# dpkn31/Yade-OpenFOAM-coupling

Measured on AMD Instinct MI355X. Metric: coupled_steps_per_sec (pimpleFoamYade 4-way, 10M particles / 4M cells per GPU), higher is better.
Workload: dtype f64

## Files before the change

yade-openfoam-coupling_amd/csrc/common.hpp:

```cpp
#pragma once
#include <hip/hip_runtime.h>

#include <algorithm>
#include <cmath>
#include <cstdarg>
#include <cstdint>
#include <cstdio>
#include <cstring>
#include <string>
#include <vector>

#include "../../include/foamyade_hip.h"

namespace fy {

struct Options {
    std::string tree_cache_dir;
    int rebin_interval;
    int strip_blocks;
    bool halo_overlap;
    int ipc_slot_mb;
    long long ipc_timeout_ms;
    bool wire_trace;
    bool explicit_tree;
    bool no_locate_lists;
    int locate_stack;
    bool locate_wide;
    bool no_deep_vcycle;
    long long mg_replicate_below;
    int amg_passes;
    bool localcomm_stream;
    bool no_fused_corrector;
    bool faces_from_arrays;
    bool no_pairs;
    bool no_tail_cache;
    int ipc_slot_kb;
};
Options options();

std::string& last_error();
int fail(int code, const char* fmt, ...);
bool pairs_disabled();
bool tail_cache_disabled();
bool locate_wide_forced();

#define FY_HIP(expr)                                                                                      \
    do {                                                                                                  \
        hipError_t _e = (expr);                                                                           \
        if (_e != hipSuccess)                                                                             \
            return ::fy::fail(FY_ERR_HIP, "%s failed: %s (%s:%d)", #expr, hipGetErrorString(_e), __FILE__, __LINE__); \
    } while (0)

#define FY_TRY(expr)                 \
    do {                             \
        int _rc = (expr);            \
        if (_rc != FY_OK) return _rc; \
    } while (0)

template <class T>
struct DevBuf {
    T* p = nullptr;
    size_t n = 0;
    DevBuf() = default;
    DevBuf(const DevBuf&) = delete;
    DevBuf& operator=(const DevBuf&) = delete;
    ~DevBuf() { release(); }
    void release() {
        if (p) (void)hipFree(p);
        p = nullptr;
        n = 0;
    }
    int reserve(size_t count) {
        if (count <= n) return FY_OK;
        release();
        size_t cap = count + count / 8 + 64;
        hipError_t e = hipMalloc((void**)&p, cap * sizeof(T));
        if (e != hipSuccess) {
            p = nullptr;
            return fail(FY_ERR_HIP, "hipMalloc(%zu bytes) failed: %s", cap * sizeof(T), hipGetErrorString(e));
        }
        n = cap;
        return FY_OK;
    }
    int alloc_exact(size_t count) {
        release();
        if (count == 0) return FY_OK;
        hipError_t e = hipMalloc((void**)&p, count * sizeof(T));
        if (e != hipSuccess) {
            p = nullptr;
            return fail(FY_ERR_HIP, "hipMalloc(%zu bytes) failed: %s", count * sizeof(T), hipGetErrorString(e));
        }
        n = count;
        return FY_OK;
    }
};

template <class T>
struct HostBuf {
    T* p = nullptr;
    size_t n = 0;
    HostBuf() = default;
    HostBuf(const HostBuf&) = delete;
    HostBuf& operator=(const HostBuf&) = delete;
    ~HostBuf() { release(); }
    void release() {
        if (p) (void)hipHostFree(p);
        p = nullptr;
        n = 0;
    }
    T* data() { return p; }
    T& operator[](size_t i) { return p[i]; }
    int reserve(size_t count) {
        if (count <= n) return FY_OK;
        release();
        const size_t cap = count + count / 8 + 64;
        hipError_t e = hipHostMalloc((void**)&p, cap * sizeof(T), hipHostMallocDefault);
        if (e != hipSuccess) {
            p = nullptr;
// ... 141 lines not shown
```

yade-openfoam-coupling_amd/csrc/coupling.cpp:

```cpp
#include "coupling.hpp"
#include "ldu.hpp"

#include <algorithm>
#include <cmath>
#include <chrono>
#include <cstdlib>
#include <functional>
#include <thread>

#include <sys/stat.h>
#include <unistd.h>

#include <atomic>

namespace fy {

static std::atomic<int> g_kernel_flags{-1};
static bool kernel_flag(int bit) {
    if (g_kernel_flags.load(std::memory_order_relaxed) < 0) (void)options();
    return (g_kernel_flags.load(std::memory_order_relaxed) >> bit) & 1;
}
bool pairs_disabled() { return kernel_flag(0); }
bool tail_cache_disabled() { return kernel_flag(1); }
bool locate_wide_forced() { return kernel_flag(2); }

Options options() {
    auto on = [](const char* nm) { const char* e = getenv(nm); return e != nullptr && *e != 0 && strcmp(e, "0") != 0; };
    auto num = [](const char* nm, long long unset) { const char* e = getenv(nm); return e ? atoll(e) : unset; };
    Options q{};
    if (const char* d = getenv("FOAMYADE_TREE_CACHE_DIR")) q.tree_cache_dir = d;
    q.rebin_interval = std::max(1, (int)num("FOAMYADE_REBIN_INTERVAL", 32));
    q.strip_blocks = (int)num("FOAMYADE_STRIP_BLOCKS", -1);
    q.halo_overlap = getenv("FOAMYADE_HALO_OVERLAP") == nullptr || on("FOAMYADE_HALO_OVERLAP");
    q.ipc_slot_mb = (int)num("FOAMYADE_IPC_SLOT_MB", 0);
    q.ipc_timeout_ms = num("FOAMYADE_IPC_TIMEOUT_MS", 0);
    q.wire_trace = getenv("FOAMYADE_WIRE_TRACE") != nullptr;
    q.explicit_tree = on("FOAMYADE_EXPLICIT_TREE");
    q.no_locate_lists = on("FOAMYADE_NO_LOCATE_LISTS");
    q.locate_stack = (int)num("FOAMYADE_LOCATE_STACK", -1);
    q.locate_wide = num("FOAMYADE_LOCATE_WIDE", 0) != 0;
    q.no_deep_vcycle = on("FOAMYADE_NO_DEEP_VCYCLE");
    q.mg_replicate_below = std::max(0LL, num("FOAMYADE_MG_REPLICATE_BELOW", 0));
    q.amg_passes = (int)std::min(3LL, std::max(1LL, num("FOAMYADE_AMG_PASSES", 3)));
    const char* ls = getenv("FOAMYADE_LOCALCOMM_STREAM");
    q.localcomm_stream = ls != nullptr && ls[0] == '1';
    q.no_fused_corrector = on("FOAMYADE_NO_FUSED_CORRECTOR");
    q.faces_from_arrays = on("FOAMYADE_FACES_FROM_ARRAYS");
    q.no_pairs = on("FOAMYADE_NO_PAIRS");
    q.no_tail_cache = on("FOAMYADE_NO_TAIL_CACHE");
    q.ipc_slot_kb = (int)num("FOAMYADE_IPC_SLOT_KB", 0);
    g_kernel_flags.store((q.no_pairs ? 1 : 0) | (q.no_tail_cache ? 2 : 0) | (q.locate_wide ? 4 : 0), std::memory_order_relaxed);
    return q;
}

std::string& last_error() {
    static thread_local std::string e;
    return e;
}

int fail(int code, const char* fmt, ...) {
    char buf[1024];
    va_list ap;
    va_start(ap, fmt);
    vsnprintf(buf, sizeof(buf), fmt, ap);
    va_end(ap);
    last_error() = buf;
    return code;
}

static const int TAG_SZ_BUFF = 1003, TAG_GRID_BBOX = 1001, TAG_YADE_DATA = 1002, TAG_FORCE = 1005, TAG_SEARCH_RES = 1004,
                 TAG_FLUID_DT = 1050, TAG_YADE_DT = 1060;

#define FY_TR(expr)                                                                             \
    do {                                                                                        \
        if ((expr) != 0) return fail(FY_ERR_TRANSPORT, "transport call failed: %s", #expr);     \
    } while (0)

int Coupling::create(const fy_mesh_desc* m, const fy_field_ptrs* f, int gaussian_interp, const fy_transport* tr, int device_ordinal) {
    if (!m || !f || m->n_cells <= 0 || !m->centres || !m->volumes) return fail(FY_ERR_INVALID, "fy_create: bad mesh/fields");
    int ndev = 0;
    if (hipGetDeviceCount(&ndev) != hipSuccess || ndev == 0)
        return fail(FY_ERR_NO_DEVICE, "no HIP device visible: libfoamyade_hip has no CPU path");
    if (device_ordinal < 0 || device_ordinal >= ndev) return fail(FY_ERR_INVALID, "device ordinal %d out of range (%d devices)", device_ordinal, ndev);
    device = device_ordinal;
    opt = options();
    FY_HIP(hipSetDevice(device));
    if (ext_stream) { stream = ext_stream; owns_stream = false; }
    else { FY_HIP(hipStreamCreate(&stream)); owns_stream = true; }
    mesh = *m;
    mesh.centres = nullptr; mesh.volumes = nullptr; mesh.xf = mesh.yf = mesh.zf = nullptr;
    n_cells = m->n_cells;
    gaussian = gaussian_interp != 0;
    structured = m->nx > 0;
    rectilinear = structured && m->xf && m->yf && m->zf;
    if (!gaussian && !structured && !ldu_geo) return fail(FY_ERR_UNSUPPORTED, "point-force mode needs the structured block description, or a general mesh's face addressing (fy_ldu_solver): the findCell stand-ins");
    if (structured && (int64_t)m->nx * m->ny * m->nz != m->n_cells) return fail(FY_ERR_INVALID, "nx*ny*nz != n_cells");
    if (tr) { transport = *tr; has_transport = true; }

    if (has_transport) {
        comm_sz_diff = std::abs(transport.world_size - transport.local_size);
        serial_yade = (comm_sz_diff == 1);
    } else {
        comm_sz_diff = 0; serial_yade = true;
    }

    {
        bool exact = structured && !rectilinear && !opt.explicit_tree && m->nx <= 1024 && m->ny <= 1024 && m->nz <= 4096 &&
                     n_cells < (1 << 25);
        if (exact)
            for (int k = 0; k < m->nz && exact; ++k) for (int j = 0; j < m->ny && exact; ++j) for (int i = 0; i < m->nx; ++i) {
                const size_t c = (size_t)i + (size_t)m->nx * (j + (size_t)m->ny * k);
                const double x = m->origin[0] + ((double)i + 0.5) * m->dx, y = m->origin[1] + ((double)j + 0.5) * m->dx, z = m->origin[2] + ((double)k + 0.5) * m->dx;
                if (x != m->centres[3 * c] || y != m->centres[3 * c + 1] || z != m->centres[3 * c + 2]) { exact = false; break; }
            }
        std::vector<int32_t> pre;
        std::string cache;
        const std::string& cache_dir = opt.tree_cache_dir;
        if (exact && !cache_dir.empty()) {
            char nm[512];
            snprintf(nm, sizeof(nm), "%s/fy_tree_%dx%dx%d_%016llx.bin", cache_dir.c_str(), m->nx, m->ny, m->nz,
                     (unsigned long long)(std::hash<double>()(m->dx) ^ (std::hash<double>()(m->origin[0]) << 1) ^ (std::hash<double>()(m->origin[1]) << 2) ^ (std::hash<double>()(m->origin[2]) << 3)));
            cache = nm;
        }
        auto load_cache = [&]() -> bool {
            FILE* f = fopen(cache.c_str(), "rb");
            if (!f) return false;
            pre.resize((size_t)n_cells);
            bool ok = fread(pre.data(), sizeof(int32_t), (size_t)n_cells, f) == (size_t)n_cells && fgetc(f) == EOF;
            fclose(f);
            for (size_t q = 0; ok && q < pre.size(); ++q) ok = pre[q] >= 0 && pre[q] < n_cells;
            if (!ok) pre.clear();
            return ok;
// ... 1306 lines not shown
```

yade-openfoam-coupling_amd/csrc/fv_kernels.hip:

```cpp
#include "fv_kernels.hpp"

#include "common.hpp"
#include "device_util.hpp"
#include "fv_closures.hpp"

#ifndef FY_FVK_GRADED
#define FY_FVK_GRADED 0
#endif

namespace fy {
#if FY_FVK_GRADED
namespace gr {
#endif
namespace {

constexpr double kSmall = 1e-15;

__device__ __forceinline__ void ijk_of(const FvGeo& g, int t, int& i, int& j, int& k) {
    i = t % g.nx;
    const int q = t / g.nx;
    j = q % g.ny;
    k = q / g.ny;
}
__device__ __forceinline__ int cidx(const FvGeo& g, int i, int j, int k) { return i + g.nx * (j + g.ny * (k + g.gz)); }
// ... 1270 lines not shown
#pragma unroll
        for (int d = 0; d < 3; ++d)
#pragma unroll
            for (int s = 0; s < 2; ++s) {
                pn[d][s] = p[nb[d][s]];
                phh[d][s] = phiHbyA.a[d][fx[d][s]];
                pfo[d][s] = pim ? phiForces.a[d][fx[d][s]] : 0.0;
                if (FFC) { rfv[d][s] = rAU[nb[d][s]]; afv[d][s] = pim ? alpha[nb[d][s]] : 1.0; }
                else { rfv[d][s] = rAUf.arr.a[d][fx[d][s]]; afv[d][s] = pim ? alphaf.arr.a[d][fx[d][s]] : 1.0; }
            }
        double pfl[3][2], ph[3][2];
#pragma unroll
        for (int d = 0; d < 3; ++d)
#pragma unroll
            for (int s = 0; s < 2; ++s) {
                const int q = ijk[d] + s;
                const int fi = i + (d == 0 ? s : 0), fj = j + (d == 1 ? s : 0), fk = k + (d == 2 ? s : 0);
                const bool b = bnd[d][s];
                if (FFC) {
                    afv[d][s] = pim ? (b ? 1.0 : lerp_face(g, d, s, q, ac, afv[d][s])) : 1.0;
                    rfv[d][s] = b ? rc : lerp_face(g, d, s, q, rc, rfv[d][s]);
                }
                const double af = afv[d][s], rf = rfv[d][s];
                double fl = 0.0;
                if (b) {
                    const int patch = 2 * d + s;
                    if (g.p_bc[patch] == 1) { const double gb = kBfac * af * rf * geo_sfd_face(g, d, q, ndim(g, d), fi, fj, fk); fl = s ? gb * (g.p_val[patch] - pc) : gb * (pc - g.p_val[patch]); }
                    else if (g.p_bc[patch] == 2) fl = af * rf * geo_Af(g, d, fi, fj, fk) * psn.a[d][fx[d][s]];
                } else {
                    fl = af * rf * geo_sfd_face(g, d, q, ndim(g, d), fi, fj, fk) * (s ? pn[d][s] - pc : pc - pn[d][s]);
                }
                const double fa = fl / af;
                pfl[d][s] = pim ? (pfo[d][s] - fa) / rf : fl;
                ph[d][s] = phh[d][s] - fa;
                if (owns_face(g, d, s, i, j, k)) phi.a[d][fx[d][s]] = ph[d][s];
            }
        double out[3];
        double dv = 0.0, sp = 0.0;
#pragma unroll
        for (int d = 0; d < 3; ++d) {
            if (!pim) {
                double fv[2];
#pragma unroll
                for (int s = 0; s < 2; ++s) {
                    if (bnd[d][s]) fv[s] = pbv(g, p, psn, c, d, s, fx[d][s]);
                    else fv[s] = geo_lerp_side(g, d, s, ijk[d], pc, pn[d][s]);
                }
                out[d] = hb[d] - rc * ((fv[1] - fv[0]) * geo_rh(g, d, ijk[d]));
            } else {
                double sm = 0;
#pragma unroll
                for (int s = 0; s < 2; ++s) sm += pfl[d][s];
                out[d] = hb[d] + rc * (sm / (2.0 * geo_Af(g, d, i, j, k)));
            }
            if (DIAG) {
#pragma unroll
                for (int s = 0; s < 2; ++s) {
                    dv += (s ? 1.0 : -1.0) * (pim ? afv[d][s] : 1.0) * ph[d][s];
                    sp += fabs(ph[d][s]);
                }
            }
        }
        for (int d = 0; d < 3; ++d) U[3 * (size_t)c + d] = out[d];
        if (DIAG) {
            double ce = dv * geo_rV(g, i, j, k);
            if (pim) ce += (ac - alphaOld[c]) / g.dt;
            v[0] += fabs(ce) * geo_V(g, i, j, k);
            v[1] += ce * geo_V(g, i, j, k);
            v[2] = fmax(v[2], sp * geo_rV(g, i, j, k));
            v[3] += sp;
        }
    }
    if (DIAG) {
        const int mx[4] = {0, 0, 1, 0};
        block_reduce_store<4>(v, mx, partials, fy_lb, fy_stride);
    }
}

template <bool STORE_A, bool FFC>
__global__ __launch_bounds__(256) __attribute__((amdgpu_waves_per_eu(4))) void k_corr_front(FvGeo g, const double* __restrict__ HbyA, const double* __restrict__ U, CFace3 dcorr,
                                                    FaceSrc rAUf, FaceSrc alphaf, CFace3 phiForces, Face3 phiHbyA, Face3 psn,
                                                    const double* __restrict__ rAU, const double* __restrict__ alpha, const double* __restrict__ alphaOld, PMat A,
                                                    double* __restrict__ rhs, const double* __restrict__ x, const double* __restrict__ xbar_dev, double xsum_val,
                                                    double inv_n, double* __restrict__ res, double* __restrict__ partials) {
    double v[2] = {0, 0};
    const double xbar = (xbar_dev ? xbar_dev[0] : xsum_val) * inv_n;
    FY_RED_LOOP_G(g, t) {
        int i, j, k; ijk_of(g, t, i, j, k);
        const int c = t + g.c0;
        const int ijk[3] = {i, j, k};
        const bool pim = g.pimple != 0;
        const bool refc = g.need_ref && (i + g.nx * (j + g.ny * (k + g.kglob0))) == g.p_ref_cell;
        bool bnd[3][2]; int nb[3][2], fx[3][2];
#pragma unroll
        for (int d = 0; d < 3; ++d)
#pragma unroll
            for (int s = 0; s < 2; ++s) {
                bnd[d][s] = onb(g, d, s, i, j, k);
                nb[d][s] = bnd[d][s] ? c : c + (s ? stride_of(g, d) : -stride_of(g, d));
                fx[d][s] = cface(g, d, s, i, j, k);
            }
        const double xc = x[c], ac = pim ? alpha[c] : 1.0;
        const double rc = FFC ? rAU[c] : 0.0;
        const double hb[3] = {HbyA[3 * (size_t)c], HbyA[3 * (size_t)c + 1], HbyA[3 * (size_t)c + 2]};
        double hn[3][2], dc[3][2], pfo[3][2], xn[3][2], rfv[3][2], afv[3][2];
#pragma unroll
        for (int d = 0; d < 3; ++d)
#pragma unroll
            for (int s = 0; s < 2; ++s) {
                hn[d][s] = HbyA[3 * (size_t)nb[d][s] + d];
                dc[d][s] = dcorr.a[d][fx[d][s]];
                pfo[d][s] = pim ? phiForces.a[d][fx[d][s]] : 0.0;
                xn[d][s] = x[nb[d][s]];
                if (FFC) { rfv[d][s] = rAU[nb[d][s]]; afv[d][s] = pim ? alpha[nb[d][s]] : 1.0; }
                else { rfv[d][s] = rAUf.arr.a[d][fx[d][s]]; afv[d][s] = pim ? alphaf.arr.a[d][fx[d][s]] : 1.0; }
            }
        double dg = 0.0, r = 0.0, up[3] = {0, 0, 0};
        double gg6[3][2];
#pragma unroll
        for (int d = 0; d < 3; ++d)
#pragma unroll
            for (int s = 0; s < 2; ++s) {
                const int q = ijk[d] + s;
                const int fi = i + (d == 0 ? s : 0), fj = j + (d == 1 ? s : 0), fk = k + (d == 2 ? s : 0);
                const bool b = bnd[d][s];
                const int patch = 2 * d + s;
                if (FFC) {
                    afv[d][s] = pim ? (b ? 1.0 : lerp_face(g, d, s, q, ac, afv[d][s])) : 1.0;
                    rfv[d][s] = b ? rc : lerp_face(g, d, s, q, rc, rfv[d][s]);
                }
                const double af = afv[d][s], rf = rfv[d][s];
                const double Afc = geo_Af(g, d, fi, fj, fk);
                double pv = (b ? ub_normal(g, patch, d, hb[d]) : lerp_face(g, d, s, q, hb[d], hn[d][s])) * Afc;
                double add = rf * dc[d][s];
                if (pim) add *= af;
                pv += add;
                if (pim) pv += pfo[d][s];
                const bool own = owns_face(g, d, s, i, j, k);
                if (own) phiHbyA.a[d][fx[d][s]] = pv;
                double ph = (s ? 1.0 : -1.0) * af * pv;
                gg6[d][s] = 0.0;
                if (b) {
                    if (g.p_bc[patch] == 2) {
                        const double ubd = ub_normal(g, patch, d, g.u_bc[patch] == 1 ? U[3 * (size_t)c + d] : 0.0);
                        const double psn_v = (pv - ubd * Afc) / (rf * Afc);
                        if (own) psn.a[d][fx[d][s]] = psn_v;
                        ph = (s ? 1.0 : -1.0) * af * (pv - rf * geo_Af(g, d, i, j, k) * psn_v);
                    }
                    r -= ph;
                    if (g.p_bc[patch] == 1) { const double gb = kBfac * af * rf * geo_sfd(g, d, s, i, j, k); dg += gb; r += gb * g.p_val[patch]; }
                } else {
                    r -= ph;
                    const double gg = af * rf * geo_sfd(g, d, s, i, j, k);
                    dg += gg; gg6[d][s] = gg;
                    if (s) up[d] = gg;
                }
            }
        if (pim) r -= geo_V(g, i, j, k) * (ac - alphaOld[c]) / g.dt;
        if (refc) { r += dg * g.p_ref_value; dg += dg; }
        if (STORE_A) { A.diag[c] = dg; A.ux[c] = up[0]; A.uy[c] = up[1]; A.uz[c] = up[2]; }
        rhs[c] = r;
        double Ax = dg * xc, rs = dg;
#pragma unroll
        for (int d = 0; d < 3; ++d)
#pragma unroll
            for (int s = 0; s < 2; ++s)
                if (!bnd[d][s]) { Ax -= gg6[d][s] * xn[d][s]; rs -= gg6[d][s]; }
        const double Aref = rs * xbar;
        const double rr = r - Ax;
        res[c] = rr;
        v[0] += fabs(rr);
        v[1] += fabs(Ax - Aref) + fabs(r - Aref);
    }
    const int mx[2] = {0, 0};
    block_reduce_store<2>(v, mx, partials, fy_lb, fy_stride);
}

__device__ __forceinline__ bool bface_side(const FvGeo& g, int b, int& side, int& r) {
    const int nyz = g.ny * g.nz, nxz = g.nx * g.nz, nxy = g.nx * g.ny;
    if (b < 2 * nyz) { side = b >= nyz; r = b - side * nyz; return true; }
    b -= 2 * nyz;
    if (b < 2 * nxz) { const int s = b >= nxz; side = 2 + s; r = b - s * nxz; return true; }
    b -= 2 * nxz;
    if (b < 2 * nxy) { const int s = b >= nxy; side = 4 + s; r = b - s * nxy; return true; }
    return false;
}
__device__ __forceinline__ double Tbv(const TPatch& e, const double* T, int c, int patch) { return e.bc[patch] == 1 ? e.val[patch] : T[c]; }
struct BFace { double A, phi, p, ux, uy, uz, T; };
template <int D, int S>
__device__ __forceinline__ void bface_values(const FvGeo& g, int r, int want, const double* __restrict__ p, const double* psn_d, const double* __restrict__ U,
                                             const double* __restrict__ T, const TPatch& te, const double* phi_d, BFace& o) {
    CFace3 psn{};
    psn.a[D] = psn_d;
    int i, j, k;
    if (D == 0) { j = r % g.ny; k = r / g.ny; i = S ? g.nx - 1 : 0; }
    else if (D == 1) { i = r % g.nx; k = r / g.nx; j = S ? g.ny - 1 : 0; }
    else { i = r % g.nx; j = r / g.nx; k = S ? g.nz - 1 : 0; }
    const int c = cidx(g, i, j, k), face = cface(g, D, S, i, j, k), patch = 2 * D + S;
    o.A = geo_Af(g, D, i, j, k);
    if (want & (1 << MF_PHI)) o.phi = (S ? 1.0 : -1.0) * phi_d[face];
    if (want & (1 << MF_P)) o.p = pbv(g, p, psn, c, D, S, face);
    if (want & (7 << MF_U)) { double u[3]; Ub(g, U, c, patch, u); o.ux = u[0]; o.uy = u[1]; o.uz = u[2]; }
    if (want & (1 << MF_T)) o.T = Tbv(te, T, c, patch);
}
__device__ __forceinline__ void bface_values_of(const FvGeo& g, int side, int r, int want, const double* __restrict__ p, CFace3 psn, const double* __restrict__ U,
                                                const double* __restrict__ T, const TPatch& te, CFace3 phi, BFace& o) {
    switch (side) {
        case 0: bface_values<0, 0>(g, r, want, p, psn.a[0], U, T, te, phi.a[0], o); break;
        case 1: bface_values<0, 1>(g, r, want, p, psn.a[0], U, T, te, phi.a[0], o); break;
        case 2: bface_values<1, 0>(g, r, want, p, psn.a[1], U, T, te, phi.a[1], o); break;
        case 3: bface_values<1, 1>(g, r, want, p, psn.a[1], U, T, te, phi.a[1], o); break;
        case 4: bface_values<2, 0>(g, r, want, p, psn.a[2], U, T, te, phi.a[2], o); break;
        default: bface_values<2, 1>(g, r, want, p, psn.a[2], U, T, te, phi.a[2], o); break;
    }
}

__global__ __launch_bounds__(256) void k_boundary_values(FvGeo g, const double* __restrict__ p, CFace3 psn, const double* __restrict__ U, const double* __restrict__ T, TPatch te,
                                                         double* __restrict__ pb, double* __restrict__ ub, double* __restrict__ tb) {
    const int b = blockIdx.x * 256 + threadIdx.x;
    int side, r;
    if (!bface_side(g, b, side, r)) return;
    BFace v{};
    bface_values_of(g, side, r, (pb ? 1 << MF_P : 0) | (ub ? 7 << MF_U : 0) | (tb ? 1 << MF_T : 0), p, psn, U, T, te, CFace3{}, v);
    if (pb) pb[b] = v.p;
    if (ub) { ub[3 * (size_t)b] = v.ux; ub[3 * (size_t)b + 1] = v.uy; ub[3 * (size_t)b + 2] = v.uz; }
    if (tb) tb[b] = v.T;
}

__global__ __launch_bounds__(256) void k_monitor_faces(FvGeo g, MonFaceTable t, const double* __restrict__ p, CFace3 psn, const double* __restrict__ U, const double* __restrict__ T,
                                                       TPatch te, CFace3 phi, double* __restrict__ partials) {
    const MonFaceObj o = t.o[blockIdx.y];
    const int b = blockIdx.x * 256 + threadIdx.x;
    int side = 0, r = 0;
    bool in = bface_side(g, b, side, r);
    in = in && ((o.patch >> side) & 1);
    BFace v{};
    if (in) bface_values_of(g, side, r, o.fields | (1 << MF_PHI), p, psn, U, T, te, phi, v);
    const double x[kMonFaceComps] = {1.0, v.phi, v.p, v.ux, v.uy, v.uz, v.T};
    const int slot0 = (int)blockIdx.y * kMonFaceComps * kMonKinds;
#pragma unroll
    for (int q = 0; q < kMonFaceComps; ++q) {
        if (!((o.fields >> q) & 1)) continue;
        double w[kMonKinds];
        mon_terms(in, x[q], v.A, v.phi, w);
        mon_block_reduce_store(w, partials, slot0 + q * kMonKinds, (int)gridDim.x, (int)blockIdx.x);
    }
}

inline int fv_grid(const FvGeo& g) { return g.win_nblk > 0 ? g.win_nblk : div_up(g.Nc, 256); }
inline int fv_red_grid(const FvGeo& g) { return g.win_nblk > 0 ? g.win_nblk : red_blocks(g.Nc); }

}

// ... 111 lines not shown

int launch_HbyA(hipStream_t s, FvGeo g, Mom7 M, const double* src, const double* U, const double* rAU, double* HbyA) {
    hipLaunchKernelGGL(k_HbyA, dim3(fv_grid(g)), dim3(256), 0, s, g, M, src, U, rAU, HbyA);
    FY_LAUNCH_CHECK();
    return FY_OK;
}

int launch_phiHbyA(hipStream_t s, FvGeo g, const double* HbyA, const double* U, const double* Uold, CFace3 phiOld, CFace3 rAUf,
                   CFace3 alphaf, CFace3 phiForces, Face3 out, Face3 psn, Face3 ddtc, int keep) {
    if (keep == 1) hipLaunchKernelGGL(k_phiHbyA_cells<1>, dim3(fv_grid(g)), dim3(256), 0, s, g, HbyA, U, Uold, phiOld, rAUf, alphaf, phiForces, out, psn, ddtc);
    else if (keep == 2) hipLaunchKernelGGL(k_phiHbyA_cells<2>, dim3(fv_grid(g)), dim3(256), 0, s, g, HbyA, U, Uold, phiOld, rAUf, alphaf, phiForces, out, psn, ddtc);
    else hipLaunchKernelGGL(k_phiHbyA_cells<0>, dim3(fv_grid(g)), dim3(256), 0, s, g, HbyA, U, Uold, phiOld, rAUf, alphaf, phiForces, out, psn, ddtc);
    FY_LAUNCH_CHECK();
    return FY_OK;
}

int launch_adjust_phi_sums(hipStream_t s, FvGeo g, CFace3 phiHbyA, CFace3 phiForces, double* partials) {
    hipLaunchKernelGGL(k_adjust_phi_sums, dim3(fv_red_grid(g)), dim3(256), 0, s, g, phiHbyA, phiForces, partials);
    FY_LAUNCH_CHECK();
    return FY_OK;
}

int launch_adjust_phi_apply(hipStream_t s, FvGeo g, const double* sums, Face3 phiHbyA, CFace3 phiForces, CFace3 rAUf, const double* U, Face3 psn, int* err) {
    const size_t nbf = 2 * ((size_t)g.ny * g.nz + (size_t)g.nx * g.nz + (size_t)g.nx * g.ny);
    hipLaunchKernelGGL(k_adjust_phi_apply, dim3(div_up(nbf, 256)), dim3(256), 0, s, g, sums, phiHbyA, phiForces, rAUf, U, psn, err);
    FY_LAUNCH_CHECK();
    return FY_OK;
}

int launch_rAUf_phi_forces(hipStream_t s, FvGeo g, const double* rAU, const double* uSource, Face3 rf, Face3 out) {
    hipLaunchKernelGGL(k_rAUf_phi_forces_cells, dim3(fv_grid(g)), dim3(256), 0, s, g, rAU, uSource, rf, out);
    FY_LAUNCH_CHECK();
    return FY_OK;
}

int launch_assemble_pressure(hipStream_t s, FvGeo g, CFace3 phiHbyA, CFace3 rAUf, CFace3 alphaf, CFace3 psn, const double* alpha,
                             const double* alphaOld, PMat A, double* rhs, bool matrix) {
    if (matrix) hipLaunchKernelGGL(k_assemble_pressure<true>, dim3(fv_grid(g)), dim3(256), 0, s, g, phiHbyA, rAUf, alphaf, psn, alpha, alphaOld, A, rhs);
    else hipLaunchKernelGGL(k_assemble_pressure<false>, dim3(fv_grid(g)), dim3(256), 0, s, g, phiHbyA, rAUf, alphaf, psn, alpha, alphaOld, A, rhs);
    FY_LAUNCH_CHECK();
    return FY_OK;
}

int launch_flux_correct(hipStream_t s, FvGeo g, const double* p, CFace3 phiHbyA, CFace3 rAUf, CFace3 alphaf, CFace3 psn, CFace3 phiForces, Face3 pflux, Face3 phi) {
    hipLaunchKernelGGL(k_flux_correct_cells, dim3(fv_grid(g)), dim3(256), 0, s, g, p, phiHbyA, rAUf, alphaf, psn, phiForces, pflux, phi);
    FY_LAUNCH_CHECK();
    return FY_OK;
}

int launch_cont_err(hipStream_t s, FvGeo g, CFace3 phi, CFace3 alphaf, const double* alpha, const double* alphaOld, double* partials) {
    hipLaunchKernelGGL(k_cont_err, dim3(fv_red_grid(g)), dim3(256), 0, s, g, phi, alphaf, alpha, alphaOld, partials);
    FY_LAUNCH_CHECK();
    return FY_OK;
}

int launch_U_correct(hipStream_t s, FvGeo g, const double* HbyA, const double* rAU, const double* p, CFace3 psn, CFace3 phiForces,
                     CFace3 pflux, CFace3 alphaf, CFace3 rAUf, double* U) {
    hipLaunchKernelGGL(k_U_correct<false>, dim3(fv_red_grid(g)), dim3(256), 0, s, g, HbyA, rAU, p, psn, phiForces, pflux, alphaf, rAUf, U, CFace3{}, nullptr, nullptr, nullptr);
    FY_LAUNCH_CHECK();
    return FY_OK;
}

int launch_U_correct_diag(hipStream_t s, FvGeo g, const double* HbyA, const double* rAU, const double* p, CFace3 psn, CFace3 phiForces,
                          CFace3 pflux, CFace3 alphaf, CFace3 rAUf, double* U, CFace3 phi, const double* alpha, const double* alphaOld, double* partials) {
    hipLaunchKernelGGL(k_U_correct<true>, dim3(fv_red_grid(g)), dim3(256), 0, s, g, HbyA, rAU, p, psn, phiForces, pflux, alphaf, rAUf, U, phi, alpha, alphaOld, partials);
    FY_LAUNCH_CHECK();
    return FY_OK;
}

int launch_corr_back(hipStream_t s, FvGeo g, const double* p, CFace3 phiHbyA, CFace3 rAUf, CFace3 alphaf, CFace3 psn, CFace3 phiForces, Face3 phi,
                     const double* HbyA, const double* rAU, double* U, const double* alpha, const double* alphaOld, double* partials, bool faces_from_cells) {
    const FaceSrc rs{rAUf, faces_from_cells ? rAU : nullptr}, as{alphaf, faces_from_cells ? alpha : nullptr};
    const dim3 grid(fv_red_grid(g)), blk(256);
#define FY_BACK(DG, FC) hipLaunchKernelGGL((k_corr_back<DG, FC>), grid, blk, 0, s, g, p, phiHbyA, rs, as, psn, phiForces, phi, HbyA, rAU, U, alpha, alphaOld, partials)
    if (partials) { if (faces_from_cells) FY_BACK(true, true); else FY_BACK(true, false); }
    else { if (faces_from_cells) FY_BACK(false, true); else FY_BACK(false, false); }
#undef FY_BACK
    FY_LAUNCH_CHECK();
    return FY_OK;
}

int launch_corr_front(hipStream_t s, FvGeo g, const double* HbyA, const double* U, CFace3 dcorr, CFace3 rAUf, CFace3 alphaf, CFace3 phiForces, Face3 phiHbyA,
                      Face3 psn, const double* rAU, const double* alpha, const double* alphaOld, PMat A, double* rhs, bool store_A, const double* x,
                      const double* xsum_dev, double xsum_val, double inv_n, double* res, double* partials, bool faces_from_cells) {
    const FaceSrc rs{rAUf, faces_from_cells ? rAU : nullptr}, as{alphaf, faces_from_cells ? alpha : nullptr};
    const dim3 grid(fv_red_grid(g)), blk(256);
#define FY_FRONT(SA, FC) hipLaunchKernelGGL((k_corr_front<SA, FC>), grid, blk, 0, s, g, HbyA, U, dcorr, rs, as, phiForces, phiHbyA, psn, rAU, alpha, alphaOld, A, rhs, \
                                            x, xsum_dev, xsum_val, inv_n, res, partials)
    if (store_A) { if (faces_from_cells) FY_FRONT(true, true); else FY_FRONT(true, false); }
    else { if (faces_from_cells) FY_FRONT(false, true); else FY_FRONT(false, false); }
#undef FY_FRONT
    FY_LAUNCH_CHECK();
    return FY_OK;
}

int launch_p_ghost_uz(hipStream_t s, FvGeo g, CFace3 rAUf, CFace3 alphaf, PMat A) {
    hipLaunchKernelGGL(k_p_ghost_uz, dim3(div_up((size_t)g.nx * g.ny, 256)), dim3(256), 0, s, g, rAUf, alphaf, A);
    FY_LAUNCH_CHECK();
    return FY_OK;
}

int launch_boundary_values(hipStream_t s, FvGeo g, const double* p, CFace3 psn, const double* U, const double* T, TPatch te, double* pb, double* ub, double* tb) {
    const size_t nb = 2 * ((size_t)g.ny * g.nz + (size_t)g.nx * g.nz + (size_t)g.nx * g.ny);
    hipLaunchKernelGGL(k_boundary_values, dim3(div_up(nb, 256)), dim3(256), 0, s, g, p, psn, U, T, te, pb, ub, tb);
    FY_LAUNCH_CHECK();
    return FY_OK;
}

int launch_monitor_faces(hipStream_t s, FvGeo g, MonFaceTable t, const double* p, CFace3 psn, const double* U, const double* T, TPatch te, CFace3 phi, double* partials, int nblk) {
    if (t.n <= 0) return FY_OK;
    hipLaunchKernelGGL(k_monitor_faces, dim3(nblk, t.n), dim3(256), 0, s, g, t, p, psn, U, T, te, phi, partials);
    FY_LAUNCH_CHECK();
    return FY_OK;
}

#if FY_FVK_GRADED
}
#endif
}
```

yade-openfoam-coupling_amd/csrc/fv_kernels_api.inc:

```

int launch_flux_of(hipStream_t s, FvGeo g, const double* F, Face3 out);
int launch_courant(hipStream_t s, FvGeo g, CFace3 phi, double* partials);
int launch_pre_coupling(hipStream_t s, FvGeo g, const double* U, const double* p, const double* alpha, CFace3 psn,
                        double* vGrad, double* gradP, double* divT, double* Gout, int write_vgrad, int write_pfields,
                        CFace3 phi = CFace3{}, double* ddtU = nullptr, double* Uold_out = nullptr,
                        double* cellrec = nullptr ,
                        double rec_nu = 0.0, double rec_rhoF = 0.0,
                        Face3 dcorr = Face3{} );
int launch_interp_alpha(hipStream_t s, FvGeo g, const double* alpha, Face3 alphaf);
int launch_div_G(hipStream_t s, FvGeo g, const double* G, double* divG);
int launch_assemble_turb(hipStream_t s, FvGeo g, TurbEqn e, const double* k, const double* eps, const double* alpha, CFace3 alphaf, CFace3 phi,
                         const double* vGrad, const double* U, Mom7 M, double* b3, double* x3);
int launch_turb_finish(hipStream_t s, FvGeo g, TurbEqn e, const double* x3, double* X, int nut_mode, double cmu, const double* eps, double* nut);
int launch_assemble_scalar(hipStream_t s, FvGeo g, ScalarEqn e, const double* T, const double* alpha, CFace3 phi, const double* Sp, const double* Su, Mom7 M,
                           double* b3, double* x3);
int launch_scalar_finish(hipStream_t s, FvGeo g, const double* x3, double* X);
int launch_smagorinsky_nut(hipStream_t s, FvGeo g, const double* vGrad, double ck, double ce, double delta, double* nut);
int launch_assemble_momentum(hipStream_t s, FvGeo g, const double* U, const double* Uold, const double* alpha, const double* alphaOld,
                             CFace3 alphaf, CFace3 phi, const double* uSource, const double* uSourceDrag, const double* divG,
                             const double* vGrad , Mom7 M, double* src, double* rAU);
int launch_grad_magsqr(hipStream_t s, FvGeo g, const double* U, double* gradL);
int launch_interp_rAU(hipStream_t s, FvGeo g, const double* rAU, Face3 rAUf);
int launch_adjust_phi_sums(hipStream_t s, FvGeo g, CFace3 phiHbyA, CFace3 phiForces, double* partials);
int launch_adjust_phi_apply(hipStream_t s, FvGeo g, const double* sums, Face3 phiHbyA, CFace3 phiForces, CFace3 rAUf, const double* U, Face3 psn, int* err);
int launch_rAUf_phi_forces(hipStream_t s, FvGeo g, const double* rAU, const double* uSource, Face3 rf, Face3 out);
int launch_bmom(hipStream_t s, FvGeo g, const double* src, const double* p, CFace3 psn, CFace3 phiForces, CFace3 rAUf, double* bmom);
int launch_bmom_faces(hipStream_t s, FvGeo g, const double* rAU, const double* uSource, const double* src, const double* p, CFace3 psn, Face3 rAUf_out,
                      Face3 phiForces, double* bmom);
int launch_mom_pass(hipStream_t s, FvGeo g, Mom7 M, const double* b, const double* x, double* xn, const double* xsum ,
                    double n_glob, double* partials, const double* hsrc = nullptr, const double* rAU = nullptr, double* HbyA = nullptr);
int launch_HbyA(hipStream_t s, FvGeo g, Mom7 M, const double* src, const double* U, const double* rAU, double* HbyA);
int launch_phiHbyA(hipStream_t s, FvGeo g, const double* HbyA, const double* U, const double* Uold, CFace3 phiOld, CFace3 rAUf,
                   CFace3 alphaf, CFace3 phiForces, Face3 phiHbyA, Face3 psn, Face3 ddtc = Face3{} ,
                   int keep = 0 );
int launch_assemble_pressure(hipStream_t s, FvGeo g, CFace3 phiHbyA, CFace3 rAUf, CFace3 alphaf, CFace3 psn, const double* alpha,
                             const double* alphaOld, PMat A, double* rhs, bool matrix = true );
int launch_flux_correct(hipStream_t s, FvGeo g, const double* p, CFace3 phiHbyA, CFace3 rAUf, CFace3 alphaf, CFace3 psn, CFace3 phiForces ,
                        Face3 pflux , Face3 phi);
int launch_cont_err(hipStream_t s, FvGeo g, CFace3 phi, CFace3 alphaf, const double* alpha, const double* alphaOld, double* partials);
int launch_U_correct(hipStream_t s, FvGeo g, const double* HbyA, const double* rAU, const double* p, CFace3 psn, CFace3 phiForces,
                     CFace3 pflux, CFace3 alphaf, CFace3 rAUf, double* U);
int launch_U_correct_diag(hipStream_t s, FvGeo g, const double* HbyA, const double* rAU, const double* p, CFace3 psn, CFace3 phiForces,
                          CFace3 pflux, CFace3 alphaf, CFace3 rAUf, double* U, CFace3 phi, const double* alpha, const double* alphaOld, double* partials);

int launch_corr_back(hipStream_t s, FvGeo g, const double* p, CFace3 phiHbyA, CFace3 rAUf, CFace3 alphaf, CFace3 psn, CFace3 phiForces, Face3 phi,
                     const double* HbyA, const double* rAU, double* U, const double* alpha, const double* alphaOld, double* partials, bool faces_from_cells);
int launch_corr_front(hipStream_t s, FvGeo g, const double* HbyA, const double* U, CFace3 dcorr, CFace3 rAUf, CFace3 alphaf, CFace3 phiForces, Face3 phiHbyA,
                      Face3 psn, const double* rAU, const double* alpha, const double* alphaOld, PMat A, double* rhs, bool store_A, const double* x,
                      const double* xsum_dev, double xsum_val, double inv_n, double* res, double* partials, bool faces_from_cells);


int launch_p_ghost_uz(hipStream_t s, FvGeo g, CFace3 rAUf, CFace3 alphaf, PMat A);
int launch_boundary_values(hipStream_t s, FvGeo g, const double* p, CFace3 psn, const double* U, const double* T, TPatch te, double* pb, double* ub, double* tb);
int launch_monitor_faces(hipStream_t s, FvGeo g, MonFaceTable t, const double* p, CFace3 psn, const double* U, const double* T, TPatch te, CFace3 phi, double* partials, int nblk);
```

yade-openfoam-coupling_amd/csrc/fv_linalg_kernels.hip:

```cpp
#include "fv_linalg_kernels.hpp"

#include "device_util.hpp"

namespace fy {
namespace {

__global__ __launch_bounds__(1024) void k_reduce_finalize(const double* __restrict__ partials, int nblocks, const int* __restrict__ ops,
                                                          double* __restrict__ out, unsigned long long* flag, unsigned long long seq) {
    __shared__ double sh[16];
    const int slot = blockIdx.x;
    const int mx = ops ? ops[slot] : 0;
    double x = mx ? -1e300 : 0.0;
    for (int b = threadIdx.x; b < nblocks; b += 1024) {
        const double y = partials[(size_t)slot * nblocks + b];
        x = mx ? fmax(x, y) : x + y;
    }
    const int lane = threadIdx.x & 63, wv = threadIdx.x >> 6;
#pragma unroll
    for (int o = 32; o > 0; o >>= 1) {
        const double y = __shfl_down(x, o, 64);
        x = mx ? fmax(x, y) : x + y;
    }
    if (lane == 0) sh[wv] = x;
    __syncthreads();
    if (threadIdx.x == 0) {
        double r = sh[0];
        for (int w = 1; w < 16; ++w) r = mx ? fmax(r, sh[w]) : r + sh[w];
        out[slot] = r;
        if (flag) {
            __threadfence_system();
            __hip_atomic_store(&flag[slot], seq, __ATOMIC_RELEASE, __HIP_MEMORY_SCOPE_SYSTEM);
        }
    }
}

__global__ __launch_bounds__(256) void k_sum3(const double* __restrict__ x, int n, double* __restrict__ partials) {
    double v[3] = {0, 0, 0};
    FY_RED_LOOP(c, n)
        for (int q = 0; q < 3; ++q) v[q] += x[3 * (size_t)c + q];
    const int mx[3] = {0, 0, 0};
    block_reduce_store<3>(v, mx, partials);
}

__device__ __forceinline__ double p_row(const PMat& A, const double* __restrict__ x, int c) {
    const int sy = A.nx, sz = A.nx * A.ny, last = A.ntot - 1;
    const int xm = max(c - 1, 0), xp = min(c + 1, last), ym = max(c - sy, 0), yp = min(c + sy, last), zm = max(c - sz, 0), zp = min(c + sz, last);
    const double uxc = A.ux[c], uyc = A.uy[c], uzc = A.uz[c];
    const double t0 = A.ux[xm] * x[xm], t1 = uxc * x[xp], t2 = A.uy[ym] * x[ym], t3 = uyc * x[yp], t4 = A.uz[zm] * x[zm], t5 = uzc * x[zp];
    double a = A.diag[c] * x[c];
    a = (c >= 1) ? a - t0 : a;
    a = (c + 1 < A.ntot) ? a - t1 : a;
    a = (c >= sy) ? a - t2 : a;
    a = (c + sy < A.ntot) ? a - t3 : a;
    a = (c >= sz) ? a - t4 : a;
    a = (c + sz < A.ntot) ? a - t5 : a;
    return a;
}
__device__ __forceinline__ double p_rowsum(const PMat& A, int c) {
    const int sy = A.nx, sz = A.nx * A.ny;
    double rs = A.diag[c];
    if (c >= 1) rs -= A.ux[c - 1];
    if (c + 1 < A.ntot) rs -= A.ux[c];
    if (c >= sy) rs -= A.uy[c - sy];
    if (c + sy < A.ntot) rs -= A.uy[c];
    if (c >= sz) rs -= A.uz[c - sz];
    if (c + sz < A.ntot) rs -= A.uz[c];
    return rs;
}

__global__ __launch_bounds__(256) void k_p_apply(PMat A, const double* __restrict__ x, double* __restrict__ y) {
    const int t = swz_block(blockIdx.x, gridDim.x) * 256 + threadIdx.x;
    if (t >= A.N) return;
    const int c = t + A.c0;
    y[c] = p_row(A, x, c);
}

template <bool WITH_R>
__global__ __launch_bounds__(256) void k_p_apply_dot(PMat A, const double* __restrict__ x, const double* __restrict__ r, double* __restrict__ y, double* __restrict__ partials) {
    double v[2] = {0, 0};
    FY_RED_LOOP(t, A.N) {
        const int c = t + A.c0;
        const double a = p_row(A, x, c);
        y[c] = a;
        const double xc = x[c];
        if (WITH_R) v[0] += xc * r[c];
        v[1] += a * xc;
    }
    if (WITH_R) {
        const int mx[2] = {0, 0};
        block_reduce_store<2>(v, mx, partials);
    } else {
        double v1[1] = {v[1]};
        const int mx[1] = {0};
        block_reduce_store<1>(v1, mx, partials + gridDim.x);
    }
}

__global__ __launch_bounds__(256) void k_p_init(PMat A, const double* __restrict__ b, const double* __restrict__ x, const double* __restrict__ xbar_dev,
                                                double xsum_val, double inv_n, double* __restrict__ r, double* __restrict__ partials) {
    double v[2] = {0, 0};
    const double xbar = (xbar_dev ? xbar_dev[0] : xsum_val) * inv_n;
    FY_RED_LOOP(t, A.N) {
        const int c = t + A.c0;
        const double Ax = p_row(A, x, c);
        const double Aref = p_rowsum(A, c) * xbar;
        const double rr = b[c] - Ax;
        r[c] = rr;
        v[0] += fabs(rr);
        v[1] += fabs(Ax - Aref) + fabs(b[c] - Aref);
    }
    const int mx[2] = {0, 0};
    block_reduce_store<2>(v, mx, partials);
}

__global__ __launch_bounds__(256) void k_dot(int n, int c0, const double* __restrict__ a, const double* __restrict__ b, double* __restrict__ partials) {
    double v[1] = {0};
    FY_RED_LOOP(t, n) v[0] += a[t + c0] * (b ? b[t + c0] : 1.0);
    const int mx[1] = {0};
    block_reduce_store<1>(v, mx, partials);
}

template <bool FIRST>
__global__ __launch_bounds__(256) void k_pcg_cg_update(int n, int c0, const double* __restrict__ u, const double* __restrict__ w, double* __restrict__ p,
                                                       double* __restrict__ sv, double* __restrict__ x, double* __restrict__ r, double* __restrict__ sc, int it,
                                                       double* __restrict__ partials) {
    double v[2] = {0, 0};
    const double gamma = sc[0], delta = sc[1];
    double beta = 0.0, al = gamma / delta;
    if (!FIRST) {
        const double gold = sc[2 + 2 * (it & 1)], aold = sc[3 + 2 * (it & 1)];
        beta = gamma / gold;
        al = gamma / (delta - beta * gamma / aold);
    }
    if (blockIdx.x == 0 && threadIdx.x == 0) { sc[2 + 2 * ((it + 1) & 1)] = gamma; sc[3 + 2 * ((it + 1) & 1)] = al; }
    FY_RED_LOOP(t, n) {
        const int c = t + c0;
        double pn = u[c], sn = w[c];
        if (!FIRST) {
            pn = pn + beta * p[c]; sn = sn + beta * sv[c];
            p[c] = pn; sv[c] = sn;
        }
        const double xn = x[c] + al * pn;
        x[c] = xn;
        const double rr = r[c] - al * sn;
        r[c] = rr;
        v[0] += fabs(rr);
        v[1] += xn;
    }
    const int mx[2] = {0, 0};
    block_reduce_store<2>(v, mx, partials);
}

__global__ __launch_bounds__(256) void k_jacobi_precond(PMat A, const double* __restrict__ r, double* __restrict__ z) {
    const int t = blockIdx.x * 256 + threadIdx.x;
    if (t < A.N) { const int c = t + A.c0; z[c] = r[c] / A.diag[c]; }
}

__global__ __launch_bounds__(256) void k_mg_coarsen(PMat F, PMat C, int ref_c, const double* __restrict__ ref_term) {
    const int tc = blockIdx.x * 256 + threadIdx.x;
    if (tc >= C.N) return;
    const int I = tc % C.nx, q = tc / C.nx, J = q % C.ny, K = q / C.ny;
    double dg = 0, ux = 0, uy = 0, uz = 0;
    for (int dk = 0; dk < 2; ++dk) {
        const int k = 2 * K + dk; if (k >= F.nz) break;
        for (int dj = 0; dj < 2; ++dj) {
            const int j = 2 * J + dj; if (j >= F.ny) break;
            for (int di = 0; di < 2; ++di) {
                const int i = 2 * I + di; if (i >= F.nx) break;
                const int c = F.c0 + i + F.nx * (j + F.ny * k);
                dg += 0.5 * F.diag[c];
                if (di == 0 && i + 1 < F.nx) dg -= F.ux[c]; else ux += 0.5 * F.ux[c];
                if (dj == 0 && j + 1 < F.ny) dg -= F.uy[c]; else uy += 0.5 * F.uy[c];
                if (dk == 0 && k + 1 < F.nz) dg -= F.uz[c]; else uz += 0.5 * F.uz[c];
            }
        }
    }
    if (tc == ref_c) dg += 0.5 * ref_term[0];
    const int cc = tc + C.c0;
    C.diag[cc] = dg; C.ux[cc] = ux; C.uy[cc] = uy; C.uz[cc] = uz;
}

__global__ void k_mg_ref_term(PMat A0, int ref_local, double* __restrict__ out) {
    if (threadIdx.x == 0 && blockIdx.x == 0) out[0] = ref_local >= 0 ? 0.5 * A0.diag[A0.c0 + ref_local] : 0.0;
}

__global__ __launch_bounds__(256) void k_mg_coarsen_ghost(PMat F, PMat C) {
    const int t = blockIdx.x * 256 + threadIdx.x;
    if (t >= C.nx * C.ny) return;
    const int I = t % C.nx, J = t / C.nx;
    double uz = 0;
    for (int dj = 0; dj < 2; ++dj) {
        const int j = 2 * J + dj; if (j >= F.ny) break;
        for (int di = 0; di < 2; ++di) {
            const int i = 2 * I + di; if (i >= F.nx) break;
            uz += 0.5 * F.uz[F.c0 - F.nx * F.ny + i + F.nx * j];
        }
    }
    C.uz[C.c0 - C.nx * C.ny + t] = uz;
}

__global__ __launch_bounds__(256) void k_mg_smooth_first(PMat A, const double* __restrict__ b, double* __restrict__ x, double w) {
    const int t = blockIdx.x * 256 + threadIdx.x;
    if (t < A.N) { const int c = t + A.c0; x[c] = w * b[c] / A.diag[c]; }
}

__global__ __launch_bounds__(256) void k_mg_smooth_two_from_zero(PMat A, const double* __restrict__ b, double* __restrict__ xn, double w, double w2) {
    const int t = blockIdx.x * 256 + threadIdx.x;
    if (t >= A.N) return;
    const int c = t + A.c0;
    const int sy = A.nx, sz = A.nx * A.ny, last = A.ntot - 1;
    const int xm = max(c - 1, 0), xp = min(c + 1, last), ym = max(c - sy, 0), yp = min(c + sy, last), zm = max(c - sz, 0), zp = min(c + sz, last);
    const double dc = A.diag[c], bc = b[c];
    const double x1c = w * bc / dc;
    const double t0 = A.ux[xm] * (w * b[xm] / A.diag[xm]), t1 = A.ux[c] * (w * b[xp] / A.diag[xp]);
    const double t2 = A.uy[ym] * (w * b[ym] / A.diag[ym]), t3 = A.uy[c] * (w * b[yp] / A.diag[yp]);
    const double t4 = A.uz[zm] * (w * b[zm] / A.diag[zm]), t5 = A.uz[c] * (w * b[zp] / A.diag[zp]);
    double a = dc * x1c;
    a = (c >= 1) ? a - t0 : a;
    a = (c + 1 < A.ntot) ? a - t1 : a;
    a = (c >= sy) ? a - t2 : a;
    a = (c + sy < A.ntot) ? a - t3 : a;
    a = (c >= sz) ? a - t4 : a;
    a = (c + sz < A.ntot) ? a - t5 : a;
    xn[c] = x1c + w2 * (bc - a) / dc;
}

__global__ __launch_bounds__(256) void k_mg_smooth_dot(PMat A, const double* __restrict__ b, const double* __restrict__ x, double* __restrict__ xn, double w,
                                                       double* __restrict__ partials) {
    double v[1] = {0};
    FY_RED_LOOP(t, A.N) {
        const int c = t + A.c0;
        const double bc = b[c];
        const double z = x[c] + w * (bc - p_row(A, x, c)) / A.diag[c];
        xn[c] = z;
        v[0] += z * bc;
    }
    const int mx[1] = {0};
    block_reduce_store<1>(v, mx, partials);
}
__global__ __launch_bounds__(256) void k_mg_smooth(PMat A, const double* __restrict__ b, const double* __restrict__ x, double* __restrict__ xn, double w) {
    const int t = swz_block(blockIdx.x, gridDim.x) * 256 + threadIdx.x;
    if (t >= A.N) return;
    const int c = t + A.c0;
    xn[c] = x[c] + w * (b[c] - p_row(A, x, c)) / A.diag[c];
}

__global__ __launch_bounds__(256) void k_mg_smooth_prolong(PMat A, const double* __restrict__ b, const double* __restrict__ x, PMat C,
                                                           const double* __restrict__ xc, double* __restrict__ xn, double w) {
    const int c = swz_block(blockIdx.x, gridDim.x) * 256 + threadIdx.x;
    if (c >= A.N) return;
    const int i = c % A.nx, q = c / A.nx, j = q % A.ny, k = q / A.ny;
    const int sy = A.nx, sz = A.nx * A.ny, last = A.ntot - 1;
    const int I = i >> 1, J = j >> 1, K = k >> 1;
    const int Im = max(i - 1, 0) >> 1, Ip = min(i + 1, A.nx - 1) >> 1, Jm = max(j - 1, 0) >> 1, Jp = min(j + 1, A.ny - 1) >> 1,
              Km = max(k - 1, 0) >> 1, Kp = min(k + 1, A.nz - 1) >> 1;
    const double* e = xc + C.c0;
    const int rowc = C.nx * (J + C.ny * K);
    const int xm = max(c - 1, 0), xp = min(c + 1, last), ym = max(c - sy, 0), yp = min(c + sy, last), zm = max(c - sz, 0), zp = min(c + sz, last);
    const double vc = x[c] + e[I + rowc];
    const double vxm = x[xm] + e[Im + rowc], vxp = x[xp] + e[Ip + rowc];
    const double vym = x[ym] + e[I + C.nx * (Jm + C.ny * K)], vyp = x[yp] + e[I + C.nx * (Jp + C.ny * K)];
    const double vzm = x[zm] + e[I + C.nx * (J + C.ny * Km)], vzp = x[zp] + e[I + C.nx * (J + C.ny * Kp)];
    const double uxc = A.ux[c], uyc = A.uy[c], uzc = A.uz[c];
    const double t0 = A.ux[xm] * vxm, t1 = uxc * vxp, t2 = A.uy[ym] * vym, t3 = uyc * vyp, t4 = A.uz[zm] * vzm, t5 = uzc * vzp;
    const double dg = A.diag[c];
    double a = dg * vc;
    a = (c >= 1) ? a - t0 : a;
    a = (c + 1 < A.ntot) ? a - t1 : a;
    a = (c >= sy) ? a - t2 : a;
    a = (c + sy < A.ntot) ? a - t3 : a;
    a = (c >= sz) ? a - t4 : a;
    a = (c + sz < A.ntot) ? a - t5 : a;
    xn[c] = vc + w * (b[c] - a) / dg;
}

__global__ __launch_bounds__(256) void k_mg_residual_restrict(PMat A, const double* __restrict__ b, const double* __restrict__ x, PMat C,
                                                              double* __restrict__ bc) {
    const int tc = blockIdx.x * 256 + threadIdx.x;
    if (tc >= C.N) return;
    const int I = tc % C.nx, q = tc / C.nx, J = q % C.ny, K = q / C.ny;
    double acc = 0;
    for (int dk = 0; dk < 2; ++dk) {
        const int k = 2 * K + dk; if (k >= A.nz) break;
        for (int dj = 0; dj < 2; ++dj) {
            const int j = 2 * J + dj; if (j >= A.ny) break;
            for (int di = 0; di < 2; ++di) {
                const int i = 2 * I + di; if (i >= A.nx) break;
                const int c = A.c0 + i + A.nx * (j + A.ny * k);
                acc += b[c] - p_row(A, x, c);
            }
        }
    }
    bc[tc + C.c0] = acc;
}

__global__ __launch_bounds__(256) void k_mg_residual_restrict_tiled(PMat A, const double* __restrict__ b, const double* __restrict__ x, PMat C,
                                                                    double* __restrict__ bc) {
    __shared__ double r[2][2][64];
    const int tx = threadIdx.x & 63, ty = (threadIdx.x >> 6) & 1, tz = threadIdx.x >> 7;
    const int i = blockIdx.x * 64 + tx, j = blockIdx.y * 2 + ty, k = blockIdx.z * 2 + tz;
    double v = 0.0;
    if (i < A.nx && j < A.ny && k < A.nz) {
        const int c = A.c0 + i + A.nx * (j + A.ny * k);
        v = b[c] - p_row(A, x, c);
    }
    r[tz][ty][tx] = v;
    __syncthreads();
    if (threadIdx.x < 32) {
        const int I = blockIdx.x * 32 + (int)threadIdx.x, J = blockIdx.y, K = blockIdx.z;
        if (I < C.nx) {
            const int q = 2 * (int)threadIdx.x;
            bc[C.c0 + I + C.nx * (J + C.ny * K)] = ((r[0][0][q] + r[0][0][q + 1]) + (r[0][1][q] + r[0][1][q + 1])) +
                                                   ((r[1][0][q] + r[1][0][q + 1]) + (r[1][1][q] + r[1][1][q + 1]));
        }
    }
}

__device__ __forceinline__ double2 ld2(const double* p) { return *reinterpret_cast<const double2*>(p); }
__device__ __forceinline__ void st2(double* p, double a, double b) { *reinterpret_cast<double2*>(p) = make_double2(a, b); }
struct PairIdx { int c, ym, yp, zm, zp, xm, xp; };
__device__ __forceinline__ PairIdx pair_idx(const PMat& A, int c) {
    const int sy = A.nx, sz = A.nx * A.ny, last = A.ntot - 1;
    return PairIdx{c, max(c - sy, 0), min(c + sy, last - 1), max(c - sz, 0), min(c + sz, last - 1), max(c - 1, 0), min(c + 2, last)};
}
struct P2 { double2 c, ym, yp, zm, zp; double xm, xp; };
__device__ __forceinline__ P2 ld_p2(const double* __restrict__ f, const PairIdx& q) {
    return P2{ld2(f + q.c), ld2(f + q.ym), ld2(f + q.yp), ld2(f + q.zm), ld2(f + q.zp), f[q.xm], f[q.xp]};
}
struct C2 { double2 dg, ux, uy, uz, uym, uzm; double uxm; };
__device__ __forceinline__ C2 ld_c2(const PMat& A, const PairIdx& q) {
    return C2{ld2(A.diag + q.c), ld2(A.ux + q.c), ld2(A.uy + q.c), ld2(A.uz + q.c), ld2(A.uy + q.ym), ld2(A.uz + q.zm), A.ux[q.xm]};
}
__device__ __forceinline__ double2 pair_rows(const PMat& A, const C2& K, const P2& X, int c) {
    const int sy = A.nx, sz = A.nx * A.ny, d = c + 1;
    double a = K.dg.x * X.c.x;
    a = (c >= 1) ? a - K.uxm * X.xm : a;
    a = (c + 1 < A.ntot) ? a - K.ux.x * X.c.y : a;
    a = (c >= sy) ? a - K.uym.x * X.ym.x : a;
    a = (c + sy < A.ntot) ? a - K.uy.x * X.yp.x : a;
    a = (c >= sz) ? a - K.uzm.x * X.zm.x : a;
    a = (c + sz < A.ntot) ? a - K.uz.x * X.zp.x : a;
    double b = K.dg.y * X.c.y;
    b = b - K.ux.x * X.c.x;
    b = (d + 1 < A.ntot) ? b - K.ux.y * X.xp : b;
    b = (d >= sy) ? b - K.uym.y * X.ym.y : b;
    b = (d + sy < A.ntot) ? b - K.uy.y * X.yp.y : b;
    b = (d >= sz) ? b - K.uzm.y * X.zm.y : b;
    b = (d + sz < A.ntot) ? b - K.uz.y * X.zp.y : b;
    return make_double2(a, b);
}
template <int N>
__device__ __forceinline__ void block_reduce_store_pairs(double2 (&v)[N], const int (&is_max)[N], double* partials, int lb = -1, int stride = 0) {
    if (lb < 0) lb = (int)blockIdx.x;
    if (stride <= 0) stride = (int)gridDim.x;
    __shared__ double sh[4][N];
    const int lane = threadIdx.x & 63, wv = threadIdx.x >> 6;
#pragma unroll
    for (int q = 0; q < N; ++q) {
        double x = v[q].x, y = v[q].y;
#pragma unroll
        for (int o = 16; o > 0; o >>= 1) {
            const double x2 = __shfl_down(x, o, 64), y2 = __shfl_down(y, o, 64);
            x = is_max[q] ? fmax(x, x2) : x + x2;
            y = is_max[q] ? fmax(y, y2) : y + y2;
        }
        if ((lane & 31) == 0) sh[2 * wv + (lane >> 5)][q] = is_max[q] ? fmax(x, y) : x + y;
    }
    __syncthreads();
    if (threadIdx.x < N) {
        const int q = threadIdx.x;
        double x = sh[0][q];
        for (int w = 1; w < 4; ++w) x = is_max[q] ? fmax(x, sh[w][q]) : x + sh[w][q];
        partials[(size_t)q * stride + lb] = x;
    }
}
#define FY_RED_LOOP2(t, n) const int t = swz_block(blockIdx.x, gridDim.x) * 256 + 2 * (int)threadIdx.x; if (t < (n))
#define FY_PAIR_LOOP(t, n) const int t = swz_block(blockIdx.x, gridDim.x) * 512 + 2 * (int)threadIdx.x; if (t < (n))

__global__ __launch_bounds__(256) void k_p_apply2(PMat A, const double* __restrict__ x, double* __restrict__ y) {
    FY_PAIR_LOOP(t, A.N) {
        const int c = t + A.c0;
        const PairIdx q = pair_idx(A, c);
        const double2 a = pair_rows(A, ld_c2(A, q), ld_p2(x, q), c);
        st2(y + c, a.x, a.y);
    }
}
template <bool WITH_R>
__global__ __launch_bounds__(128) void k_p_apply_dot2(PMat A, const double* __restrict__ x, const double* __restrict__ r, double* __restrict__ y, double* __restrict__ partials) {
    double2 v[2] = {make_double2(0, 0), make_double2(0, 0)};
    FY_RED_LOOP2(t, A.N) {
        const int c = t + A.c0;
        const PairIdx q = pair_idx(A, c);
        const P2 X = ld_p2(x, q);
        const double2 a = pair_rows(A, ld_c2(A, q), X, c);
        st2(y + c, a.x, a.y);
        if (WITH_R) { const double2 rc = ld2(r + c); v[0] = make_double2(X.c.x * rc.x, X.c.y * rc.y); }
        v[1] = make_double2(a.x * X.c.x, a.y * X.c.y);
    }
    if (WITH_R) {
        const int mx[2] = {0, 0};
        block_reduce_store_pairs<2>(v, mx, partials);
    } else {
        double2 v1[1] = {v[1]};
        const int mx[1] = {0};
        block_reduce_store_pairs<1>(v1, mx, partials + gridDim.x);
    }
}
template <bool FIRST>
__global__ __launch_bounds__(128) void k_pcg_cg_update2(int n, int c0, const double* __restrict__ u, const double* __restrict__ w, double* __restrict__ p,
                                                        double* __restrict__ sv, double* __restrict__ x, double* __restrict__ r, double* __restrict__ sc, int it,
                                                        double* __restrict__ partials) {
    double2 v[2] = {make_double2(0, 0), make_double2(0, 0)};
    const double gamma = sc[0], delta = sc[1];
    double beta = 0.0, al = gamma / delta;
    if (!FIRST) {
        const double gold = sc[2 + 2 * (it & 1)], aold = sc[3 + 2 * (it & 1)];
        beta = gamma / gold;
        al = gamma / (delta - beta * gamma / aold);
    }
    if (blockIdx.x == 0 && threadIdx.x == 0) { sc[2 + 2 * ((it + 1) & 1)] = gamma; sc[3 + 2 * ((it + 1) & 1)] = al; }
    FY_RED_LOOP2(t, n) {
        const int c = t + c0;
        double2 pn = ld2(u + c), sn = ld2(w + c);
        if (!FIRST) {
            const double2 po = ld2(p + c), so = ld2(sv + c);
            pn = make_double2(pn.x + beta * po.x, pn.y + beta * po.y); sn = make_double2(sn.x + beta * so.x, sn.y + beta * so.y);
            st2(p + c, pn.x, pn.y); st2(sv + c, sn.x, sn.y);
        }
        const double2 xo = ld2(x + c), ro = ld2(r + c);
        const double xa = xo.x + al * pn.x, xb = xo.y + al * pn.y;
        st2(x + c, xa, xb);
        const double ra = ro.x - al * sn.x, rb = ro.y - al * sn.y;
        st2(r + c, ra, rb);
        v[0] = make_double2(fabs(ra), fabs(rb));
        v[1] = make_double2(xa, xb);
    }
    const int mx[2] = {0, 0};
    block_reduce_store_pairs<2>(v, mx, partials);
}
__global__ __launch_bounds__(256) void k_mg_smooth_two_from_zero2(PMat A, const double* __restrict__ b, double* __restrict__ xn, double w, double w2) {
    const int t = (int)blockIdx.x * 512 + 2 * (int)threadIdx.x;
    if (t >= A.N) return;
    const int c = t + A.c0;
    const PairIdx q = pair_idx(A, c);
    const P2 B = ld_p2(b, q), D = ld_p2(A.diag, q);
    C2 K = ld_c2(A, q);
    K.dg = D.c;
    P2 X1;
    X1.c = make_double2(w * B.c.x / D.c.x, w * B.c.y / D.c.y);
    X1.ym = make_double2(w * B.ym.x / D.ym.x, w * B.ym.y / D.ym.y); X1.yp = make_double2(w * B.yp.x / D.yp.x, w * B.yp.y / D.yp.y);
    X1.zm = make_double2(w * B.zm.x / D.zm.x, w * B.zm.y / D.zm.y); X1.zp = make_double2(w * B.zp.x / D.zp.x, w * B.zp.y / D.zp.y);
    X1.xm = w * B.xm / D.xm; X1.xp = w * B.xp / D.xp;
    const double2 a = pair_rows(A, K, X1, c);
    st2(xn + c, X1.c.x + w2 * (B.c.x - a.x) / D.c.x, X1.c.y + w2 * (B.c.y - a.y) / D.c.y);
}
__global__ __launch_bounds__(128) void k_mg_smooth_dot2(PMat A, const double* __restrict__ b, const double* __restrict__ x, double* __restrict__ xn, double w,
                                                        double* __restrict__ partials) {
    double2 v[1] = {make_double2(0, 0)};
    FY_RED_LOOP2(t, A.N) {
        const int c = t + A.c0;
        const PairIdx q = pair_idx(A, c);
        const C2 K = ld_c2(A, q);
        const P2 X = ld_p2(x, q);
        const double2 bc = ld2(b + c), a = pair_rows(A, K, X, c);
        const double za = X.c.x + w * (bc.x - a.x) / K.dg.x, zb = X.c.y + w * (bc.y - a.y) / K.dg.y;
        st2(xn + c, za, zb);
        v[0] = make_double2(za * bc.x, zb * bc.y);
    }
    const int mx[1] = {0};
    block_reduce_store_pairs<1>(v, mx, partials);
}
__global__ __launch_bounds__(256) void k_mg_smooth2(PMat A, const double* __restrict__ b, const double* __restrict__ x, double* __restrict__ xn, double w) {
    FY_PAIR_LOOP(t, A.N) {
        const int c = t + A.c0;
        const PairIdx q = pair_idx(A, c);
        const C2 K = ld_c2(A, q);
        const P2 X = ld_p2(x, q);
        const double2 bc = ld2(b + c), a = pair_rows(A, K, X, c);
        st2(xn + c, X.c.x + w * (bc.x - a.x) / K.dg.x, X.c.y + w * (bc.y - a.y) / K.dg.y);
    }
}
__global__ __launch_bounds__(256) void k_mg_smooth_prolong2(PMat A, const double* __restrict__ b, const double* __restrict__ x, PMat C,
                                                            const double* __restrict__ xc, double* __restrict__ xn, double w) {
    FY_PAIR_LOOP(c, A.N) {
        const int i = c % A.nx, qq = c / A.nx, j = qq % A.ny, k = qq / A.ny;
        const int I = i >> 1, J = j >> 1, Kk = k >> 1;
        const int Im = max(i - 1, 0) >> 1, Ip = min(i + 2, A.nx - 1) >> 1, Jm = max(j - 1, 0) >> 1, Jp = min(j + 1, A.ny - 1) >> 1,
                  Km = max(k - 1, 0) >> 1, Kp = min(k + 1, A.nz - 1) >> 1;
        const double* e = xc + C.c0;
        const int rowc = C.nx * (J + C.ny * Kk);
        const PairIdx q = pair_idx(A, c);
        const C2 K = ld_c2(A, q);
        P2 V = ld_p2(x, q);
        const double ec = e[I + rowc], eym = e[I + C.nx * (Jm + C.ny * Kk)], eyp = e[I + C.nx * (Jp + C.ny * Kk)],
                     ezm = e[I + C.nx * (J + C.ny * Km)], ezp = e[I + C.nx * (J + C.ny * Kp)];
        V.c.x += ec; V.c.y += ec; V.ym.x += eym; V.ym.y += eym; V.yp.x += eyp; V.yp.y += eyp; V.zm.x += ezm; V.zm.y += ezm; V.zp.x += ezp; V.zp.y += ezp;
        V.xm += e[Im + rowc]; V.xp += e[Ip + rowc];
        const double2 bc = ld2(b + c), a = pair_rows(A, K, V, c);
        st2(xn + c, V.c.x + w * (bc.x - a.x) / K.dg.x, V.c.y + w * (bc.y - a.y) / K.dg.y);
    }
}
template <int PX, int TY, int TZ>
__global__ __launch_bounds__(256) void k_mg_residual_restrict_tiled2(PMat A, const double* __restrict__ b, const double* __restrict__ x, PMat C,
                                                                     double* __restrict__ bc) {
    static_assert(PX * TY * TZ == 256 && TY % 2 == 0 && TZ % 2 == 0, "tile shape");
    __shared__ double r[TZ][TY][PX];
    const int tx = threadIdx.x % PX, ty = (threadIdx.x / PX) % TY, tz = threadIdx.x / (PX * TY);
    const int i = blockIdx.x * (2 * PX) + 2 * tx, j = blockIdx.y * TY + ty, k = blockIdx.z * TZ + tz;
    double v = 0.0;
    if (i < A.nx && j < A.ny && k < A.nz) {
        const int c = A.c0 + i + A.nx * (j + A.ny * k);
        const PairIdx q = pair_idx(A, c);
        const double2 bb = ld2(b + c), a = pair_rows(A, ld_c2(A, q), ld_p2(x, q), c);
        v = (bb.x - a.x) + (bb.y - a.y);
    }
    r[tz][ty][tx] = v;
    __syncthreads();
    constexpr int NC = PX * (TY / 2) * (TZ / 2);
    if ((int)threadIdx.x < NC) {
        const int cx = threadIdx.x % PX, cy = (threadIdx.x / PX) % (TY / 2), cz = threadIdx.x / (PX * (TY / 2));
        const int I = blockIdx.x * PX + cx, J = blockIdx.y * (TY / 2) + cy, K = blockIdx.z * (TZ / 2) + cz;
        if (I < C.nx && J < C.ny && K < C.nz)
            bc[C.c0 + I + C.nx * (J + C.ny * K)] = (r[2 * cz][2 * cy][cx] + r[2 * cz][2 * cy + 1][cx]) + (r[2 * cz + 1][2 * cy][cx] + r[2 * cz + 1][2 * cy + 1][cx]);
    }
}

constexpr int kMgCoarseMax = 256;
struct MgTail {
    int n;
    PMat A[kMgTailMax];
    double* x0[kMgTailMax];
    double* x1[kMgTailMax];
    double* b[kMgTailMax];
    const double* fac;
    int cache_n, cache_off;
};

__device__ __forceinline__ double read_lane_f64(double v, int src_lane) {
    const int lo = __builtin_amdgcn_readlane(__double2loint(v), src_lane), hi = __builtin_amdgcn_readlane(__double2hiint(v), src_lane);
    return __hiloint2double(hi, lo);
}
template <bool FWD, bool LO, bool DO0, bool DO1>
__device__ __forceinline__ void band_columns(const double* Ls, int N, int bw, int ja, int jb, int lane, double& v0, double& v1) {
    if (jb <= ja) return;
    constexpr int U = 8;
    const int Wd = bw + 1, r0 = min(lane, N - 1), r1 = min(lane + 64, N - 1);
    for (int g = 0; g < jb - ja; g += U) {
        double dj[U], a0[U], a1[U];
#pragma unroll
        for (int u = 0; u < U; ++u) {
            const int jr = FWD ? ja + g + u : jb - 1 - g - u;
            const bool live = FWD ? jr < jb : jr >= ja;
            const int j = min(max(jr, 0), N - 1);
            dj[u] = live ? Ls[(size_t)j * Wd] : 0.0;
            const int d0 = FWD ? lane - jr : jr - lane, d1 = FWD ? lane + 64 - jr : jr - (lane + 64);
            a0[u] = 0.0; a1[u] = 0.0;
            if (DO0) {
                const double c0 = FWD ? Ls[(size_t)r0 * Wd + min(max(d0, 0), bw)] : Ls[(size_t)j * Wd + min(max(d0, 0), bw)];
                a0[u] = (live && d0 >= 1 && d0 <= bw && lane < N) ? c0 : 0.0;
            }
            if (DO1) {
                const double c1 = FWD ? Ls[(size_t)r1 * Wd + min(max(d1, 0), bw)] : Ls[(size_t)j * Wd + min(max(d1, 0), bw)];
                a1[u] = (live && d1 >= 1 && d1 <= bw && lane + 64 < N) ? c1 : 0.0;
            }
        }
#pragma unroll
        for (int u = 0; u < U; ++u) {
            const int jr = FWD ? ja + g + u : jb - 1 - g - u;
            const int j = min(max(jr, 0), N - 1);
            const double yj = read_lane_f64(LO ? v0 : v1, j & 63) * dj[u];
            if (DO0) v0 -= a0[u] * yj;
            if (DO1) v1 -= a1[u] * yj;
        }
    }
}
__device__ __forceinline__ void coarse_band_solve(const double* Ls, int N, int bw, const double* __restrict__ b, double* __restrict__ x, int lane) {
    const int Wd = bw + 1;
    double v0 = lane < N ? b[lane] : 0.0, v1 = lane + 64 < N ? b[lane + 64] : 0.0;
    const double dg0 = Ls[(size_t)min(lane, N - 1) * Wd], dg1 = Ls[(size_t)min(lane + 64, N - 1) * Wd];
    const int n0 = min(N, 64);
    const int js = min(max(64 - bw, 0), n0);
    band_columns<true, true, true, false>(Ls, N, bw, 0, js, lane, v0, v1);
    band_columns<true, true, true, true>(Ls, N, bw, js, n0, lane, v0, v1);
    band_columns<true, false, false, true>(Ls, N, bw, 64, N, lane, v0, v1);
    v0 *= dg0; v1 *= dg1;
    const int jt = min(64 + bw, N);
    band_columns<false, false, false, true>(Ls, N, bw, jt, N, lane, v0, v1);
    band_columns<false, false, true, true>(Ls, N, bw, 64, jt, lane, v0, v1);
    band_columns<false, true, true, false>(Ls, N, bw, 0, n0, lane, v0, v1);
    v0 *= dg0; v1 *= dg1;
    if (lane < N) x[lane] = v0;
    if (lane + 64 < N) x[lane + 64] = v1;
}

__global__ __launch_bounds__(1024) void k_mg_tail(MgTail T, double w, int coarse_sweeps, MgWeights W) {
    const int tid = threadIdx.x;
    extern __shared__ double tail_lds[];
    const bool cached = T.cache_n > 0;
    double* const lc = tail_lds + T.cache_off;
    PMat AL = T.A[0];
    if (cached) {
        const int N0 = T.cache_n;
        AL.diag = lc; AL.ux = lc + N0; AL.uy = lc + 2 * N0; AL.uz = lc + 3 * N0;
        for (int c = tid; c < N0; c += 1024) {
            AL.diag[c] = T.A[0].diag[c]; AL.ux[c] = T.A[0].ux[c]; AL.uy[c] = T.A[0].uy[c]; AL.uz[c] = T.A[0].uz[c];
            lc[4 * N0 + c] = T.b[0][c];
// ... 215 lines not shown
        double* t = cur; cur = nxt; nxt = t;
    }
    if (cur != x) { if (act) x[c] = cur[c]; }
}

__global__ __launch_bounds__(256) void k_relax_field(double* __restrict__ x, const double* __restrict__ prev, double alpha, size_t n) {
    const size_t i = (size_t)blockIdx.x * 256 + threadIdx.x;
    if (i < n) x[i] = prev[i] + alpha * (x[i] - prev[i]);
}

__global__ __launch_bounds__(256) void k_copy(double* __restrict__ dst, const double* __restrict__ src, size_t n) {
    const size_t i = (size_t)blockIdx.x * 256 + threadIdx.x;
    if (i < n) dst[i] = src[i];
}

__global__ __launch_bounds__(256) void k_add(double* __restrict__ y, const double* __restrict__ x, size_t n) {
    const size_t i = (size_t)blockIdx.x * 256 + threadIdx.x;
    if (i < n) y[i] += x[i];
}

__global__ __launch_bounds__(256) void k_buoyancy(size_t n3, const double* __restrict__ T, double beta, double T_ref, double gx, double gy, double gz,
                                                  const double* __restrict__ uSource, double* __restrict__ a_out, double* __restrict__ sum_out) {
    const size_t e = (size_t)blockIdx.x * 256 + threadIdx.x;
    if (e >= n3) return;
    const size_t c = e / 3;
    const int q = (int)(e - 3 * c);
    const double a = (-beta * (T[c] - T_ref)) * (q == 0 ? gx : q == 1 ? gy : gz);
    a_out[e] = a;
    sum_out[e] = uSource[e] + a;
}

}

int launch_buoyancy(hipStream_t s, size_t n_cells, const double* T, double beta, double T_ref, const double* g, const double* uSource, double* a, double* sum) {
    if (!n_cells) return FY_OK;
    hipLaunchKernelGGL(k_buoyancy, dim3(div_up(3 * n_cells, 256)), dim3(256), 0, s, 3 * n_cells, T, beta, T_ref, g[0], g[1], g[2], uSource, a, sum);
    FY_LAUNCH_CHECK();
    return FY_OK;
}

int launch_reduce_finalize(hipStream_t s, const double* partials, int n_cells, int nslots, const int* ops, double* out, unsigned long long* flag,
                           unsigned long long seq) {
    hipLaunchKernelGGL(k_reduce_finalize, dim3(nslots), dim3(1024), 0, s, partials, red_blocks(n_cells), ops, out, flag, seq);
    FY_LAUNCH_CHECK();
    return FY_OK;
}

int launch_sum3(hipStream_t s, const double* x, int n, double* partials) {
    hipLaunchKernelGGL(k_sum3, dim3(red_blocks(n)), dim3(256), 0, s, x, n, partials);
    FY_LAUNCH_CHECK();
    return FY_OK;
}

static bool al16(const void* p) { return (reinterpret_cast<uintptr_t>(p) & 15u) == 0; }
static bool pairs_ok(const PMat& A) {
    return !pairs_disabled() && A.N >= 2 && A.nx % 2 == 0 && A.c0 % 2 == 0 && A.N % 2 == 0 && A.ntot % 2 == 0 && al16(A.diag) && al16(A.ux) && al16(A.uy) && al16(A.uz);
}
static bool pairs_ok(int n, int c0) {
    return !pairs_disabled() && n >= 2 && n % 2 == 0 && c0 % 2 == 0;
}

int launch_p_apply(hipStream_t s, PMat A, const double* x, double* y) {
    if (pairs_ok(A) && al16(x) && al16(y)) {
        hipLaunchKernelGGL(k_p_apply2, dim3(div_up(A.N, 512)), dim3(256), 0, s, A, x, y);
        FY_LAUNCH_CHECK();
        return FY_OK;
    }
    hipLaunchKernelGGL(k_p_apply, dim3(div_up(A.N, 256)), dim3(256), 0, s, A, x, y);
    FY_LAUNCH_CHECK();
    return FY_OK;
}

int launch_p_apply_dot(hipStream_t s, PMat A, const double* x, const double* r, double* y, double* partials) {
    if (pairs_ok(A) && al16(x) && al16(y) && al16(r)) {
        if (r) hipLaunchKernelGGL(k_p_apply_dot2<true>, dim3(red_blocks(A.N)), dim3(128), 0, s, A, x, r, y, partials);
        else hipLaunchKernelGGL(k_p_apply_dot2<false>, dim3(red_blocks(A.N)), dim3(128), 0, s, A, x, r, y, partials);
    }
    else if (r) hipLaunchKernelGGL(k_p_apply_dot<true>, dim3(red_blocks(A.N)), dim3(256), 0, s, A, x, r, y, partials);
    else hipLaunchKernelGGL(k_p_apply_dot<false>, dim3(red_blocks(A.N)), dim3(256), 0, s, A, x, r, y, partials);
    FY_LAUNCH_CHECK();
    return FY_OK;
}

int launch_p_init(hipStream_t s, PMat A, const double* b, const double* x, const double* xsum_dev, double xsum_val, double inv_n, double* r, double* partials) {
    hipLaunchKernelGGL(k_p_init, dim3(red_blocks(A.N)), dim3(256), 0, s, A, b, x, xsum_dev, xsum_val, inv_n, r, partials);
    FY_LAUNCH_CHECK();
    return FY_OK;
}

int launch_dot(hipStream_t s, int n, int c0, const double* a, const double* b, double* partials) {
    hipLaunchKernelGGL(k_dot, dim3(red_blocks(n)), dim3(256), 0, s, n, c0, a, b, partials);
    FY_LAUNCH_CHECK();
    return FY_OK;
}

int launch_pcg_cg_update(hipStream_t s, int n, int c0, const double* u, const double* w, double* p, double* sv, double* x, double* r, double* sc, int it, double* partials) {
    if (pairs_ok(n, c0) && al16(u) && al16(w) && al16(p) && al16(sv) && al16(x) && al16(r)) {
        if (it == 0) hipLaunchKernelGGL(k_pcg_cg_update2<true>, dim3(red_blocks(n)), dim3(128), 0, s, n, c0, u, w, p, sv, x, r, sc, it, partials);
        else hipLaunchKernelGGL(k_pcg_cg_update2<false>, dim3(red_blocks(n)), dim3(128), 0, s, n, c0, u, w, p, sv, x, r, sc, it, partials);
    }
    else if (it == 0) hipLaunchKernelGGL(k_pcg_cg_update<true>, dim3(red_blocks(n)), dim3(256), 0, s, n, c0, u, w, p, sv, x, r, sc, it, partials);
    else hipLaunchKernelGGL(k_pcg_cg_update<false>, dim3(red_blocks(n)), dim3(256), 0, s, n, c0, u, w, p, sv, x, r, sc, it, partials);
    FY_LAUNCH_CHECK();
    return FY_OK;
}

int launch_jacobi_precond(hipStream_t s, PMat A, const double* r, double* z) {
    hipLaunchKernelGGL(k_jacobi_precond, dim3(div_up(A.N, 256)), dim3(256), 0, s, A, r, z);
    FY_LAUNCH_CHECK();
    return FY_OK;
}

int launch_mg_ref_term(hipStream_t s, PMat A0, int ref_local, double* out) {
    hipLaunchKernelGGL(k_mg_ref_term, dim3(1), dim3(64), 0, s, A0, ref_local, out);
    FY_LAUNCH_CHECK();
    return FY_OK;
}

int launch_mg_coarsen(hipStream_t s, PMat F, PMat C, int ref_c, const double* ref_term) {
    hipLaunchKernelGGL(k_mg_coarsen, dim3(div_up(C.N, 256)), dim3(256), 0, s, F, C, ref_term ? ref_c : -1, ref_term);
    FY_LAUNCH_CHECK();
    return FY_OK;
}

int launch_mg_smooth_first(hipStream_t s, PMat A, const double* b, double* x, double w) {
    hipLaunchKernelGGL(k_mg_smooth_first, dim3(div_up(A.N, 256)), dim3(256), 0, s, A, b, x, w);
    FY_LAUNCH_CHECK();
    return FY_OK;
}

int launch_mg_smooth_two_from_zero(hipStream_t s, PMat A, const double* b, double* xn, double w, double w2) {
    if (pairs_ok(A) && al16(b) && al16(xn)) hipLaunchKernelGGL(k_mg_smooth_two_from_zero2, dim3(div_up(A.N, 512)), dim3(256), 0, s, A, b, xn, w, w2);
    else hipLaunchKernelGGL(k_mg_smooth_two_from_zero, dim3(div_up(A.N, 256)), dim3(256), 0, s, A, b, xn, w, w2);
    FY_LAUNCH_CHECK();
    return FY_OK;
}

int launch_mg_smooth_dot(hipStream_t s, PMat A, const double* b, const double* x, double* xn, double w, double* partials) {
    if (pairs_ok(A) && al16(b) && al16(x) && al16(xn)) hipLaunchKernelGGL(k_mg_smooth_dot2, dim3(red_blocks(A.N)), dim3(128), 0, s, A, b, x, xn, w, partials);
    else hipLaunchKernelGGL(k_mg_smooth_dot, dim3(red_blocks(A.N)), dim3(256), 0, s, A, b, x, xn, w, partials);
    FY_LAUNCH_CHECK();
    return FY_OK;
}

int launch_mg_smooth(hipStream_t s, PMat A, const double* b, const double* x, double* xn, double w) {
    if (pairs_ok(A) && al16(b) && al16(x) && al16(xn)) hipLaunchKernelGGL(k_mg_smooth2, dim3(div_up(A.N, 512)), dim3(256), 0, s, A, b, x, xn, w);
    else hipLaunchKernelGGL(k_mg_smooth, dim3(div_up(A.N, 256)), dim3(256), 0, s, A, b, x, xn, w);
    FY_LAUNCH_CHECK();
    return FY_OK;
}

static int band_width(const PMat& A) { return A.nz > 1 ? A.nx * A.ny : (A.ny > 1 ? A.nx : 1); }
static size_t fac_lds_bytes(int N, int bw) { return (size_t)N * (size_t)(bw + 1) * sizeof(double); }
static int allow_big_lds(const void* fn) {
    return hipFuncSetAttribute(fn, hipFuncAttributeMaxDynamicSharedMemorySize, (int)fac_lds_bytes(kMgDirectMax, kMgDirectBand)) == hipSuccess ? FY_OK
           : fail(FY_ERR_HIP, "hipFuncSetAttribute(MaxDynamicSharedMemorySize) failed");
}

int mg_coarse_factor_doubles(PMat A) { return 3 + A.N * (band_width(A) + 1); }
bool mg_coarse_direct_ok(PMat A) { return A.c0 == 0 && A.N <= kMgDirectMax && band_width(A) <= kMgDirectBand; }

int launch_mg_coarse_factor(hipStream_t s, PMat A, double* fac) {
    if (!(mg_coarse_direct_ok)(A)) return fail(FY_ERR_INVALID, "direct coarse solve: level of %d cells, band %d (ghost offset %d)", A.N, band_width(A), A.c0);
    static bool attr_set = false;
    if (!attr_set) {
        FY_TRY(allow_big_lds(reinterpret_cast<const void*>(k_mg_coarse_factor<1>)));
        FY_TRY(allow_big_lds(reinterpret_cast<const void*>(k_mg_coarse_factor<2>)));
        FY_TRY(allow_big_lds(reinterpret_cast<const void*>(k_mg_coarse_factor<3>)));
        attr_set = true;
    }
    const int bw = band_width(A);
    const int tri = bw * (bw + 1) / 2;
    const int q = tri <= 1024 ? 1 : (tri <= 2048 ? 2 : 3);
    const int nt = std::min(1024, ((tri + q - 1) / q + 63) / 64 * 64);
    if (q == 1) hipLaunchKernelGGL(k_mg_coarse_factor<1>, dim3(1), dim3(nt), fac_lds_bytes(A.N, bw), s, A, bw, fac);
    else if (q == 2) hipLaunchKernelGGL(k_mg_coarse_factor<2>, dim3(1), dim3(nt), fac_lds_bytes(A.N, bw), s, A, bw, fac);
    else hipLaunchKernelGGL(k_mg_coarse_factor<3>, dim3(1), dim3(nt), fac_lds_bytes(A.N, bw), s, A, bw, fac);
    FY_LAUNCH_CHECK();
    return FY_OK;
}

int launch_mg_tail(hipStream_t s, const PMat* A, double* const* x0, double* const* x1, double* const* b, int n, double w, int coarse_sweeps, MgWeights W,
                   const double* fac) {
    if (n < 1 || n > kMgTailMax) return fail(FY_ERR_INVALID, "bad multigrid tail depth %d", n);
    MgTail T;
    T.n = n;
    T.fac = fac;
    size_t lds = 0;
    static bool attr_set = false;
    if (!attr_set) {
        const int want = (int)(fac_lds_bytes(kMgDirectMax, kMgDirectBand) + 7 * (size_t)kMgTailCells * sizeof(double));
        if (hipFuncSetAttribute(reinterpret_cast<const void*>(k_mg_tail), hipFuncAttributeMaxDynamicSharedMemorySize, want) != hipSuccess)
            return fail(FY_ERR_HIP, "hipFuncSetAttribute(MaxDynamicSharedMemorySize) failed");
        attr_set = true;
    }
    if (fac) {
        if (!(mg_coarse_direct_ok)(A[n - 1])) return fail(FY_ERR_INVALID, "multigrid tail: a factor was handed over for a level it cannot belong to");
        lds = fac_lds_bytes(A[n - 1].N, band_width(A[n - 1]));
    }
    T.cache_n = 0; T.cache_off = (int)(lds / sizeof(double));
    if (!tail_cache_disabled() && n >= 2 && A[0].N <= kMgTailCells) { T.cache_n = A[0].N; lds += 7 * (size_t)A[0].N * sizeof(double); }
    for (int l = 0; l < n; ++l) {
        if (A[l].c0 != 0) return fail(FY_ERR_INVALID, "multigrid tail levels must not carry ghost planes");
        T.A[l] = A[l]; T.x0[l] = x0[l]; T.x1[l] = x1[l]; T.b[l] = b[l];
    }
    if (W.n < 2 || (W.n & 1)) return fail(FY_ERR_INVALID, "the multigrid tail needs an even number of smoothing sweeps");
    hipLaunchKernelGGL(k_mg_tail, dim3(1), dim3(1024), lds, s, T, w, coarse_sweeps, W);
    FY_LAUNCH_CHECK();
    return FY_OK;
}

int launch_mg_residual_restrict(hipStream_t s, PMat A, const double* b, const double* x, PMat C, double* bc) {
    if (C.N > 8192 && C.ny * 2 >= A.ny && C.nz * 2 >= A.nz) {
        if (pairs_ok(A) && al16(b) && al16(x) && A.ny % 2 == 0 && A.nz % 2 == 0) {
            const int px_opts[4] = {64, 32, 16, 8};
            int best = 64; double best_fill = 0.0;
            for (int px : px_opts) { const double fill = (double)A.nx / (double)(div_up(A.nx, 2 * px) * 2 * px); if (fill > best_fill + 1e-9) { best_fill = fill; best = px; } }
            if (best == 64) hipLaunchKernelGGL((k_mg_residual_restrict_tiled2<64, 2, 2>), dim3(div_up(A.nx, 128), div_up(A.ny, 2), div_up(A.nz, 2)), dim3(256), 0, s, A, b, x, C, bc);
            else if (best == 32) hipLaunchKernelGGL((k_mg_residual_restrict_tiled2<32, 4, 2>), dim3(div_up(A.nx, 64), div_up(A.ny, 4), div_up(A.nz, 2)), dim3(256), 0, s, A, b, x, C, bc);
            else if (best == 16) hipLaunchKernelGGL((k_mg_residual_restrict_tiled2<16, 4, 4>), dim3(div_up(A.nx, 32), div_up(A.ny, 4), div_up(A.nz, 4)), dim3(256), 0, s, A, b, x, C, bc);
            else hipLaunchKernelGGL((k_mg_residual_restrict_tiled2<8, 8, 4>), dim3(div_up(A.nx, 16), div_up(A.ny, 8), div_up(A.nz, 4)), dim3(256), 0, s, A, b, x, C, bc);
        }
        else hipLaunchKernelGGL(k_mg_residual_restrict_tiled, dim3(div_up(A.nx, 64), C.ny, C.nz), dim3(256), 0, s, A, b, x, C, bc);
        FY_LAUNCH_CHECK();
        return FY_OK;
    }
    hipLaunchKernelGGL(k_mg_residual_restrict, dim3(div_up(C.N, 256)), dim3(256), 0, s, A, b, x, C, bc);
    FY_LAUNCH_CHECK();
    return FY_OK;
}

int launch_mg_smooth_prolong(hipStream_t s, PMat A, const double* b, const double* x, PMat C, const double* xc, double* xn, double w) {
    if (A.c0 != 0 || A.ntot != A.N) return fail(FY_ERR_INVALID, "k_mg_smooth_prolong works on levels without ghost planes");
    if (pairs_ok(A) && al16(b) && al16(x) && al16(xn)) hipLaunchKernelGGL(k_mg_smooth_prolong2, dim3(div_up(A.N, 512)), dim3(256), 0, s, A, b, x, C, xc, xn, w);
    else hipLaunchKernelGGL(k_mg_smooth_prolong, dim3(div_up(A.N, 256)), dim3(256), 0, s, A, b, x, C, xc, xn, w);
    FY_LAUNCH_CHECK();
    return FY_OK;
}

int launch_mg_prolong_add(hipStream_t s, PMat A, double* x, PMat C, const double* xc) {
    hipLaunchKernelGGL(k_mg_prolong_add, dim3(div_up(A.N, 256)), dim3(256), 0, s, A, x, C, xc);
    FY_LAUNCH_CHECK();
    return FY_OK;
}

int launch_mg_prolong_add_planes(hipStream_t s, PMat A, int kofs, double* x, PMat C, const double* xc) {
    hipLaunchKernelGGL(k_mg_prolong_add_planes, dim3(div_up(A.N, 256)), dim3(256), 0, s, A, kofs, x, C, xc);
    FY_LAUNCH_CHECK();
    return FY_OK;
}

int launch_mg_coarse_solve(hipStream_t s, PMat A, const double* b, double* x, double* tmp, int sweeps, double w, const double* fac) {
    if (A.c0 != 0) return fail(FY_ERR_INVALID, "the coarsest multigrid level must be replicated (no ghost planes)");
    if (A.N > 1024) return fail(FY_ERR_INVALID, "coarsest multigrid level too large (%d cells)", A.N);
    size_t lds = 0;
    if (fac) {
        if (!(mg_coarse_direct_ok)(A)) return fail(FY_ERR_INVALID, "coarse solve: a factor was handed over for a level it cannot belong to");
        static bool attr_set = false;
        if (!attr_set) { FY_TRY(allow_big_lds(reinterpret_cast<const void*>(k_mg_coarse_solve))); attr_set = true; }
        lds = fac_lds_bytes(A.N, band_width(A));
    }
    hipLaunchKernelGGL(k_mg_coarse_solve, dim3(1), dim3(1024), lds, s, A, b, x, tmp, sweeps, w, fac);
    FY_LAUNCH_CHECK();
    return FY_OK;
}

int launch_relax_field(hipStream_t s, double* x, const double* prev, double alpha, size_t n) {
    if (n == 0) return FY_OK;
    hipLaunchKernelGGL(k_relax_field, dim3(div_up(n, 256)), dim3(256), 0, s, x, prev, alpha, n);
    FY_LAUNCH_CHECK();
    return FY_OK;
}

int launch_copy_f64(hipStream_t s, double* dst, const double* src, size_t n) {
    if (!n) return FY_OK;
    hipLaunchKernelGGL(k_copy, dim3(div_up(n, 256)), dim3(256), 0, s, dst, src, n);
    FY_LAUNCH_CHECK();
    return FY_OK;
}

int launch_mg_coarsen_ghost(hipStream_t s, PMat F, PMat C) {
    hipLaunchKernelGGL(k_mg_coarsen_ghost, dim3(div_up((size_t)C.nx * C.ny, 256)), dim3(256), 0, s, F, C);
    FY_LAUNCH_CHECK();
    return FY_OK;
}

int launch_add_f64(hipStream_t s, double* y, const double* x, size_t n) {
    if (!n) return FY_OK;
    hipLaunchKernelGGL(k_add, dim3(div_up(n, 256)), dim3(256), 0, s, y, x, n);
    FY_LAUNCH_CHECK();
    return FY_OK;
}

}
```

yade-openfoam-coupling_amd/csrc/fv_linalg_kernels.hpp:

```cpp
#pragma once
#include <hip/hip_runtime.h>

#include <cstddef>

namespace fy {

struct PMat {
    int nx, ny, nz, N;
    int c0, ntot;
    double *diag, *ux, *uy, *uz;
};

inline int red_blocks(int n) { return (((n + 255) / 256) + 7) & ~7; }

constexpr int kMgDirectMax = 128, kMgDirectBand = 64;
constexpr int kMgTailMax = 6;
constexpr int kMgTailCells = 1024;
struct MgWeights { int n; double w[4]; };

int launch_reduce_finalize(hipStream_t s, const double* partials, int n_cells, int nslots, const int* ops , double* out,
                           unsigned long long* flag = nullptr, unsigned long long seq = 0);
int launch_sum3(hipStream_t s, const double* x, int n, double* partials);

int launch_p_apply(hipStream_t s, PMat A, const double* x, double* y);
int launch_p_apply_dot(hipStream_t s, PMat A, const double* x, const double* r , double* y, double* partials);
int launch_p_init(hipStream_t s, PMat A, const double* b, const double* x, const double* xsum_dev , double xsum_val, double inv_n,
                  double* r, double* partials);
int launch_dot(hipStream_t s, int n, int c0, const double* a, const double* b , double* partials);
int launch_pcg_cg_update(hipStream_t s, int n, int c0, const double* u, const double* w, double* p, double* sv, double* x, double* r, double* sc, int it, double* partials);
int launch_jacobi_precond(hipStream_t s, PMat A, const double* r, double* z);
int launch_mg_coarsen(hipStream_t s, PMat F, PMat C, int ref_c = -1, const double* ref_term = nullptr);
int launch_mg_ref_term(hipStream_t s, PMat A0, int ref_local, double* out);
int launch_mg_smooth_first(hipStream_t s, PMat A, const double* b, double* x, double w);
int launch_mg_smooth_two_from_zero(hipStream_t s, PMat A, const double* b, double* xn, double w, double w2);
int launch_mg_smooth(hipStream_t s, PMat A, const double* b, const double* x, double* xn, double w);
int launch_mg_smooth_dot(hipStream_t s, PMat A, const double* b, const double* x, double* xn, double w, double* partials);
int launch_mg_residual_restrict(hipStream_t s, PMat A, const double* b, const double* x, PMat C, double* bc);
int launch_mg_prolong_add(hipStream_t s, PMat A, double* x, PMat C, const double* xc);
int launch_mg_prolong_add_planes(hipStream_t s, PMat A , int kofs , double* x, PMat C, const double* xc);
int launch_mg_smooth_prolong(hipStream_t s, PMat A, const double* b, const double* x, PMat C, const double* xc, double* xn, double w);
bool mg_coarse_direct_ok(PMat A);
int mg_coarse_factor_doubles(PMat A);
int launch_mg_coarse_factor(hipStream_t s, PMat A, double* fac);
int launch_mg_coarse_solve(hipStream_t s, PMat A, const double* b, double* x, double* tmp, int sweeps, double w, const double* fac = nullptr);
int launch_mg_tail(hipStream_t s, const PMat* A, double* const* x0, double* const* x1, double* const* b, int n, double w, int coarse_sweeps, MgWeights W,
                   const double* fac = nullptr);

int launch_copy_f64(hipStream_t s, double* dst, const double* src, size_t n);
int launch_relax_field(hipStream_t s, double* x, const double* prev, double alpha, size_t n);
int launch_mg_coarsen_ghost(hipStream_t s, PMat F, PMat C);
int launch_add_f64(hipStream_t s, double* y, const double* x, size_t n);
int launch_buoyancy(hipStream_t s, size_t n_cells, const double* T, double beta, double T_ref, const double* g, const double* uSource, double* a, double* sum);

}
```

yade-openfoam-coupling_amd/csrc/fv_pressure.cpp:

```cpp
#include "fv_solver.hpp"

namespace fy {

int Solver::smooth(size_t l, MgLev& L, double w, bool with_dot) {
    if (L.distributed && overlap_halos && L.A.nz >= 4) {
        const int pl = (int)L.plane;
        FY_HIP(hipEventRecord(ev_ready, stream));
        FY_HIP(hipStreamWaitEvent(comm_stream, ev_ready, 0));
        PMat in = L.A; in.c0 += pl; in.N -= 2 * pl;
        FY_TRY(launch_mg_smooth(stream, in, L.bptr, L.xcur, L.xalt, w));
        FY_TRY(halo(L.xcur, 1, L.plane, L.A.nz, L.gz, 1, comm_stream));
        FY_HIP(hipEventRecord(ev_halo, comm_stream));
        FY_HIP(hipStreamWaitEvent(stream, ev_halo, 0));
        PMat lo = L.A; lo.N = pl;
        PMat hi = L.A; hi.c0 += (L.A.nz - 1) * pl; hi.N = pl;
        FY_TRY(launch_mg_smooth(stream, lo, L.bptr, L.xcur, L.xalt, w));
        FY_TRY(launch_mg_smooth(stream, hi, L.bptr, L.xcur, L.xalt, w));
        std::swap(L.xcur, L.xalt);
        return FY_OK;
    }
    FY_TRY(halo_level(L, L.xcur));
    if (with_dot) {
        if (l == 0) kc[KC_MG_SMOOTH0].begin(stream);
        FY_TRY(launch_mg_smooth_dot(stream, L.A, L.bptr, L.xcur, L.xalt, w, partials.p));
        if (l == 0) kc[KC_MG_SMOOTH0].end(stream);
        std::swap(L.xcur, L.xalt);
        return FY_OK;
    }
    if (l == 0) kc[KC_MG_SMOOTH0].begin(stream);
    FY_TRY(launch_mg_smooth(stream, L.A, L.bptr, L.xcur, L.xalt, w));
    if (l == 0) kc[KC_MG_SMOOTH0].end(stream);
    std::swap(L.xcur, L.xalt);
    return FY_OK;
}

PMat Solver::slice_of(const MgLev& L, const MgLev& Cc) const {
    PMat loc = Cc.A;
    loc.nz = L.A.nz / 2; loc.N = (int)(Cc.plane * (size_t)loc.nz); loc.c0 = 0; loc.ntot = loc.N;
    return loc;
}

PMat Solver::planes_of(const MgLev& L, int ext, int* kofs) const {
    const int lo = comm->has_down() ? -ext : 0, hi = L.A.nz + (comm->has_up() ? ext : 0);
    PMat R = L.A;
    R.c0 = L.A.c0 + lo * (int)L.plane;
    R.N = (hi - lo) * (int)L.plane;
    if (kofs) *kofs = lo;
    return R;
}

int Solver::vcycle_deep(size_t l, int E) {
    MgLev& L = *mg[l];
    MgLev& Cc = *mg[l + 1];
    const MgWeights& W = mgw;
    if (l >= 1) FY_TRY(wait_coarse());
    if (E + 3 > L.gz || E + 3 > L.A.nz) return fail(FY_ERR_INVALID, "vcycle_deep: level %zu has %d ghost planes, %d are needed", l, L.gz, E + 3);
    int kofs = 0;
    const PMat R2 = planes_of(L, E + 2, &kofs);
    if (overlap_halos && L.A.nz >= 4) {
        const int pl = (int)L.plane;
        FY_HIP(hipEventRecord(ev_ready, stream));
        FY_HIP(hipStreamWaitEvent(comm_stream, ev_ready, 0));
        FY_TRY(halo(const_cast<double*>(L.bptr), 1, L.plane, L.A.nz, L.gz, E + 3, comm_stream));
        FY_HIP(hipEventRecord(ev_halo, comm_stream));
        PMat in = L.A; in.c0 += pl; in.N -= 2 * pl;
        FY_TRY(launch_mg_smooth_two_from_zero(stream, in, L.bptr, L.xcur, W.w[0], W.w[1]));
        FY_HIP(hipStreamWaitEvent(stream, ev_halo, 0));
        PMat lo = R2; lo.N = (1 - kofs) * pl;
        PMat hi = R2; hi.c0 = L.A.c0 + (L.A.nz - 1) * pl; hi.N = R2.N - (L.A.nz - 1 - kofs) * pl;
        FY_TRY(launch_mg_smooth_two_from_zero(stream, lo, L.bptr, L.xcur, W.w[0], W.w[1]));
        FY_TRY(launch_mg_smooth_two_from_zero(stream, hi, L.bptr, L.xcur, W.w[0], W.w[1]));
    } else {
        FY_TRY(halo(const_cast<double*>(L.bptr), 1, L.plane, L.A.nz, L.gz, E + 3));
        if (l == 0) kc[KC_MG_SMOOTH0].begin(stream);
        FY_TRY(launch_mg_smooth_two_from_zero(stream, R2, L.bptr, L.xcur, W.w[0], W.w[1]));
        if (l == 0) kc[KC_MG_SMOOTH0].end(stream);
    }
    if (!Cc.distributed) {
        PMat loc = slice_of(L, Cc);
        FY_TRY(launch_mg_residual_restrict(stream, L.A, L.bptr, L.xcur, loc, rep_stage.p));
        FY_TRY(comm->allgather(stream, rep_stage.p, Cc.b.p, (size_t)loc.N));
        Cc.bptr = Cc.b.p;
        FY_TRY(vcycle(l + 1));
        PMat under = Cc.A;
        under.c0 = (int)(Cc.plane * (size_t)(L.A.nz / 2) * (size_t)comm->rank);
        FY_TRY(launch_mg_prolong_add_planes(stream, R2, kofs, L.xcur, under, Cc.xcur));
    } else {
        FY_TRY(launch_mg_residual_restrict(stream, L.A, L.bptr, L.xcur, Cc.A, Cc.b.p));
        Cc.bptr = Cc.b.p;
        FY_TRY(vcycle_deep(l + 1, (E + 3) / 2));
        FY_TRY(launch_mg_prolong_add_planes(stream, R2, kofs, L.xcur, Cc.A, Cc.xcur));
    }
    FY_TRY(launch_mg_smooth(stream, planes_of(L, E + 1), L.bptr, L.xcur, L.xalt, W.w[1]));
    std::swap(L.xcur, L.xalt);
    if (l == 0) kc[KC_MG_SMOOTH0].begin(stream);
    FY_TRY(launch_mg_smooth(stream, planes_of(L, E), L.bptr, L.xcur, L.xalt, W.w[0]));
    if (l == 0) kc[KC_MG_SMOOTH0].end(stream);
    std::swap(L.xcur, L.xalt);
    return FY_OK;
}

int Solver::vcycle(size_t l) {
    const double w = 0.8;
    const MgWeights& W = mgw;
    if (l >= 1) FY_TRY(wait_coarse());
    MgLev& L = *mg[l];
    if (!L.distributed && L.A.N <= kMgTailCells && mg.size() - l <= (size_t)kMgTailMax) {
        FY_TRY(wait_factor());
        PMat A[kMgTailMax]; double* x0[kMgTailMax]; double* x1[kMgTailMax]; double* b[kMgTailMax];
        const int n = (int)(mg.size() - l);
        for (int q = 0; q < n; ++q) {
            MgLev& M = *mg[l + (size_t)q];
            A[q] = M.A; x0[q] = M.x0.p; x1[q] = M.x1.p; b[q] = q == 0 ? const_cast<double*>(L.bptr) : M.b.p;
        }
        FY_TRY(launch_mg_tail(stream, A, x0, x1, b, n, w, coarse_sweeps, W, mg_inv.p));
        L.xcur = n > 1 ? L.x1.p : L.x0.p; L.xalt = n > 1 ? L.x0.p : L.x1.p;
        return FY_OK;
    }
    if (l + 1 == mg.size()) {
        FY_TRY(wait_factor());
        FY_TRY(launch_mg_coarse_solve(stream, L.A, L.bptr, L.x0.p, L.x1.p, coarse_sweeps, w, mg_inv.p));
        L.xcur = L.x0.p; L.xalt = L.x1.p;
        return FY_OK;
    }
    MgLev& Cc = *mg[l + 1];
    if (!L.distributed) {
        FY_TRY(launch_mg_smooth_two_from_zero(stream, L.A, L.bptr, L.xcur, W.w[0], W.w[1]));
    } else {
        FY_TRY(launch_mg_smooth_first(stream, L.A, L.bptr, L.xcur, W.w[0]));
        FY_TRY(smooth(l, L, W.w[1]));
    }
    for (int s = 2; s < W.n; ++s) FY_TRY(smooth(l, L, W.w[s]));
    FY_TRY(halo_level(L, L.xcur));
    const bool handover = L.distributed && !Cc.distributed;
    if (handover) {
        PMat loc = slice_of(L, Cc);
        FY_TRY(launch_mg_residual_restrict(stream, L.A, L.bptr, L.xcur, loc, rep_stage.p));
        FY_TRY(comm->allgather(stream, rep_stage.p, Cc.b.p, (size_t)loc.N));
    } else {
        FY_TRY(launch_mg_residual_restrict(stream, L.A, L.bptr, L.xcur, Cc.A, Cc.b.p));
    }
    Cc.bptr = Cc.b.p;
    FY_TRY(vcycle(l + 1));
    if (handover) {
        PMat loc = Cc.A;
        loc.c0 = (int)(Cc.plane * (size_t)(L.A.nz / 2) * (size_t)comm->rank);
        FY_TRY(launch_mg_prolong_add(stream, L.A, L.xcur, loc, Cc.xcur));
        for (int s = W.n - 1; s >= 1; --s) FY_TRY(smooth(l, L, W.w[s]));
    } else if (!L.distributed && W.n >= 2 && fuse_prolong) {
        FY_TRY(launch_mg_smooth_prolong(stream, L.A, L.bptr, L.xcur, Cc.A, Cc.xcur, L.xalt, W.w[W.n - 1]));
        std::swap(L.xcur, L.xalt);
        for (int s = W.n - 2; s >= 1; --s) FY_TRY(smooth(l, L, W.w[s]));
    } else {
        FY_TRY(launch_mg_prolong_add(stream, L.A, L.xcur, Cc.A, Cc.xcur));
        for (int s = W.n - 1; s >= 1; --s) FY_TRY(smooth(l, L, W.w[s]));
    }
    vcycle_dot_done = l == 0 && want_vcycle_dot && !L.distributed && L.A.N == Nc && L.A.c0 == g.c0;
    FY_TRY(smooth(l, L, W.w[0], vcycle_dot_done));
    return FY_OK;
}

int Solver::ref_cell_at(size_t lvl, const PMat& A, int k0) const {
    if (!g.need_ref) return -1;
    const int i = (g.p_ref_cell % g.nx) >> lvl, j = ((g.p_ref_cell / g.nx) % g.ny) >> lvl, k = (g.p_ref_cell / (g.nx * g.ny)) >> lvl;
    const int kl = k - k0;
    if (kl < 0 || kl >= A.nz) return -1;
    return i + A.nx * (j + A.ny * kl);
}

int Solver::exchange_operator_ghosts(MgLev& L) {
    if (!L.distributed) return FY_OK;
    comm->group_begin();
    double* arr[4] = {L.A.diag, L.A.ux, L.A.uy, L.A.uz};
    for (double* a : arr) FY_TRY(halo(a, 1, L.plane, L.A.nz, L.gz, std::min(L.gz, L.A.nz)));
    return comm->group_end(stream);
}

int Solver::build_coarse_operators() {
    Comm::Tag tag(comm, "p_operators");
    const double* ref_term = nullptr;
    if (g.need_ref && mg.size() > 1) {
        if (!mg_ref.p) FY_TRY(mg_ref.alloc_exact(1));
        FY_TRY(launch_mg_ref_term(stream, mg[0]->A, ref_cell_at(0, mg[0]->A, mg[0]->distributed ? g.kglob0 : 0), mg_ref.p));
        if (mg[0]->distributed) FY_TRY(comm->allreduce(stream, mg_ref.p, 1, false));
        ref_term = mg_ref.p;
    }
    if (mg_deep) FY_TRY(exchange_operator_ghosts(*mg[0]));
    for (size_t l = 0; l + 1 < mg.size(); ++l) {
        MgLev& F = *mg[l]; MgLev& Cc = *mg[l + 1];
        if (F.distributed && !Cc.distributed) {
            PMat loc = slice_of(F, Cc);
            const size_t cnt = (size_t)loc.N;
            loc.diag = rep_stage.p; loc.ux = rep_stage.p + cnt; loc.uy = rep_stage.p + 2 * cnt; loc.uz = rep_stage.p + 3 * cnt;
            FY_TRY(launch_mg_coarsen(stream, F.A, loc, ref_cell_at(l + 1, loc, comm->rank * loc.nz), ref_term));
            if (rep_gather.n < 4 * cnt * (size_t)comm->size) FY_TRY(rep_gather.alloc_exact(4 * cnt * (size_t)comm->size));
            FY_TRY(comm->allgather(stream, rep_stage.p, rep_gather.p, 4 * cnt));
            double* dst[4] = {Cc.A.diag, Cc.A.ux, Cc.A.uy, Cc.A.uz};
            for (int r = 0; r < comm->size; ++r)
                for (int a = 0; a < 4; ++a)
                    FY_TRY(launch_copy_f64(stream, dst[a] + (size_t)r * cnt, rep_gather.p + ((size_t)r * 4 + (size_t)a) * cnt, cnt));
        } else {
            FY_TRY(launch_mg_coarsen(stream, F.A, Cc.A, ref_cell_at(l + 1, Cc.A, Cc.distributed ? comm->rank * Cc.A.nz : 0), ref_term));
            if (Cc.distributed) {
                if (mg_deep) FY_TRY(exchange_operator_ghosts(Cc));
                else if (comm->has_down()) FY_TRY(launch_mg_coarsen_ghost(stream, F.A, Cc.A));
            }
        }
    }
    if (cs.p_solver == FY_PSOLVER_PCG_MG) {
        const MgLev& Lc = *mg.back();
        if (!Lc.distributed && mg_coarse_direct_ok(Lc.A)) {
            if (!mg_inv.p) FY_TRY(mg_inv.alloc_exact((size_t)mg_coarse_factor_doubles(Lc.A)));
            if (coarse_on_side) { FY_HIP(hipEventRecord(ev_coarse, stream)); coarse_marked = true; }
            FY_TRY(launch_mg_coarse_factor(stream, Lc.A, mg_inv.p));
        }
    }
    return FY_OK;
}

int Solver::prepare_p_init(bool with_halo) {
    if (!p_sum_valid) {
        FY_TRY(launch_dot(stream, Nc, g.c0, p.p, nullptr, partials.p));
        FY_TRY(reduce_to_device(sc.p + 6));
    }
    return with_halo ? halo_p() : FY_OK;
}

int Solver::solve_pressure(bool final_iter, bool init_done) {
    Comm::Tag tag(comm, "pcg");
    MgLev& L = *mg[0];
    const double tol = final_iter ? cs.p_final_tol : cs.p_tol, rel = final_iter ? cs.p_final_rel_tol : cs.p_rel_tol;
    double h[2];
    if (!init_done) {
        FY_TRY(prepare_p_init());
        FY_TRY(launch_p_init(stream, L.A, prhs.p, p.p, p_sum_valid ? nullptr : sc.p + 6, p_sum, 1.0 / (double)Nglob, pr.p, partials.p));
    }
    FY_TRY(reduce_read(2, false, h));
    const double norm = h[1] + 1e-20;
    double res = h[0] / norm;
    const double res0 = res;
    st.p_initial_residual = res0;
    auto converged = [&](double r) { return r < tol || (rel > 0 && r < rel * res0); };
    int it = 0;
    if (!converged(res)) {
        do {
            const double* u;
            bool u_ghosts = false;
            vcycle_dot_done = false;
            if (cs.p_solver == FY_PSOLVER_PCG_MG) {
                L.bptr = pr.p;
                Comm::Tag vt(comm, "vcycle");
                if (mg_deep) { FY_TRY(vcycle_deep(0, 1)); u_ghosts = true; }
                else { want_vcycle_dot = true; FY_TRY(vcycle(0)); want_vcycle_dot = false; }
                u = L.xcur;
            } else {
                FY_TRY(launch_jacobi_precond(stream, L.A, pr.p, pzj.p));
                u = pzj.p;
            }
            if (!u_ghosts) FY_TRY(halo(const_cast<double*>(u), 1, plane, g.nz, g.gz, 1));
            kc[KC_P_APPLY_DOT].begin(stream);
            FY_TRY(launch_p_apply_dot(stream, L.A, u, vcycle_dot_done ? nullptr : pr.p, pw.p, partials.p));
            kc[KC_P_APPLY_DOT].end(stream);
            FY_TRY(launch_reduce_finalize(stream, partials.p, Nc, 2, nullptr, sc.p));
            FY_TRY(comm->allreduce(stream, sc.p, 2, false));
            FY_TRY(launch_pcg_cg_update(stream, Nc, g.c0, u, pw.p, pp.p, ps.p, p.p, pr.p, sc.p, it, partials.p));
            if (it == 0) {
                std::swap(ps.p, pw.p);
                if (u == L.xcur) {
                    double*& held = (L.xcur == L.x0.p) ? L.x0.p : L.x1.p;
                    std::swap(pp.p, held);
                    L.xcur = held; L.xalt = (L.xcur == L.x0.p) ? L.x1.p : L.x0.p;
                } else {
                    std::swap(pp.p, pzj.p);
                }
            }
            p_ghosts_fresh = false;
            FY_TRY(reduce_read(2, false, h));
            res = h[0] / norm;
            p_sum = h[1]; p_sum_valid = true;
        } while (++it < cs.p_max_iter && !converged(res));
    }
    st.p_final_residual = res;
    st.p_iters_total += it; st.p_solves += 1;
    return FY_OK;
}

int Solver::precondition(const double* r_host, double* z_host) {
    Comm::Tag tag(comm, "vcycle");
    MgLev& L = *mg[0];
    const size_t bytes = (size_t)Nc * sizeof(double);
    const double* u;
    if (cs.p_solver == FY_PSOLVER_PCG_MG) {
        struct Roles { double* xcur; double* xalt; const double* bptr; };
        std::vector<Roles> keep;
        for (auto& M : mg) keep.push_back(Roles{M->xcur, M->xalt, M->bptr});
        const bool want = want_vcycle_dot, done = vcycle_dot_done;
        FY_HIP(hipMemcpyAsync(pzj.p + g.c0, r_host, bytes, hipMemcpyHostToDevice, stream));
        L.bptr = pzj.p;
        int rc;
        if (mg_deep) rc = vcycle_deep(0, 1);
        else { want_vcycle_dot = true; rc = vcycle(0); }
        u = L.xcur;
        if (rc == FY_OK && hipMemcpyAsync(z_host, u + g.c0, bytes, hipMemcpyDeviceToHost, stream) != hipSuccess) rc = fail(FY_ERR_HIP, "fy_solver_precondition_host: copy to the host failed");
        want_vcycle_dot = want; vcycle_dot_done = done;
        for (size_t l = 0; l < mg.size(); ++l) { mg[l]->xcur = keep[l].xcur; mg[l]->xalt = keep[l].xalt; mg[l]->bptr = keep[l].bptr; }
        FY_TRY(rc);
    } else {
        FY_HIP(hipMemcpyAsync(pw.p + g.c0, r_host, bytes, hipMemcpyHostToDevice, stream));
        FY_TRY(launch_jacobi_precond(stream, L.A, pw.p, pzj.p));
        FY_HIP(hipMemcpyAsync(z_host, pzj.p + g.c0, bytes, hipMemcpyDeviceToHost, stream));
    }
    FY_HIP(hipStreamSynchronize(stream));
    return FY_OK;
}

}
```

yade-openfoam-coupling_amd/csrc/fv_solver.cpp:

```cpp
#include "fv_solver.hpp"

namespace fy {

int Solver::create(const fy_case_desc* c, const fy_transport* tr, int dev, Comm* cm) {
    if (c && (c->convection_scheme < FY_CONVECTION_LINEAR || c->convection_scheme > FY_CONVECTION_QUICK)) return fail(FY_ERR_INVALID, "fy_solver_create: unknown convection_scheme");
    if (c && c->convection_scheme == FY_CONVECTION_LIMITED_LINEAR && !(c->convection_limiter_k >= 0 && c->convection_limiter_k <= 1)) return fail(FY_ERR_INVALID, "fy_solver_create: limitedLinear's coefficient must lie in [0, 1]");
    const bool gradedc = c && (c->hx || c->hy || c->hz);
    if (!c || c->nx <= 0 || c->ny <= 0 || c->nz <= 0 || (!gradedc && !(c->dx > 0)) || !(c->dt > 0)) return fail(FY_ERR_INVALID, "fy_solver_create: bad case");
    if (gradedc) {
        if (!(c->hx && c->hy && c->hz)) return fail(FY_ERR_INVALID, "fy_solver_create: a graded block needs hx, hy AND hz");
        if (cm && cm->size > 1) return fail(FY_ERR_UNSUPPORTED, "fy_solver_create: z-slabs need the uniform block (a graded block runs on one domain)");
        const double* hh[3] = {c->hx, c->hy, c->hz};
        const int nn[3] = {c->nx, c->ny, c->nz};
        for (int a = 0; a < 3; ++a) for (int q = 0; q < nn[a]; ++q) if (!(hh[a][q] > 0)) return fail(FY_ERR_INVALID, "fy_solver_create: graded block with a non-positive cell size");
    }
    if (c->thermal.on && cm && cm->size > 1)
        return fail(FY_ERR_UNSUPPORTED, "fy_solver_create_slab: heat transfer (fy_case_desc.thermal.on) is not available on z-slabs (%d ranks; foamYadeHip_mpi -parallel): "
                                        "run the case on one domain", cm->size);
    int ndev = 0;
    if (hipGetDeviceCount(&ndev) != hipSuccess || ndev == 0) return fail(FY_ERR_NO_DEVICE, "no HIP device visible: libfoamyade_hip has no CPU path");
    if (dev < 0 || dev >= ndev) return fail(FY_ERR_INVALID, "device ordinal out of range");
    cs = *c; device = dev; pimple = c->solver == FY_SOLVER_PIMPLE;
    cs.hx = cs.hy = cs.hz = nullptr;
    comm = cm ? cm : &self_comm;
    FY_HIP(hipSetDevice(device));
    FY_HIP(hipStreamCreate(&stream));
    FY_HIP(hipStreamCreateWithFlags(&comm_stream, hipStreamNonBlocking));
    FY_HIP(hipEventCreateWithFlags(&ev_ready, hipEventDisableTiming));
    FY_HIP(hipEventCreateWithFlags(&ev_halo, hipEventDisableTiming));
    FY_HIP(hipEventCreateWithFlags(&ev_assembled, hipEventDisableTiming));
    FY_HIP(hipEventCreateWithFlags(&ev_usum0, hipEventDisableTiming));
    FY_HIP(hipEventCreateWithFlags(&ev_usum1, hipEventDisableTiming));
    FY_HIP(hipEventCreateWithFlags(&ev_coarse, hipEventDisableTiming));
    FY_HIP(hipEventCreateWithFlags(&ev_factor, hipEventDisableTiming));
    const Options opt = options();
    overlap_halos = opt.halo_overlap;
    fused_corrector = !opt.no_fused_corrector;
    faces_from_cells = !opt.faces_from_arrays;
    comm->set_aux_stream(comm_stream);
    const int S = comm->size;
    if (c->nz % S != 0) return fail(FY_ERR_INVALID, "nz (%d) must be divisible by the number of slabs (%d)", c->nz, S);
    const int nzl = c->nz / S;
    if (S > 1 && (nzl % 2 != 0 || nzl < 2)) return fail(FY_ERR_INVALID, "each slab needs an even number (>= 2) of z-planes, got %d", nzl);
    const int gz = S == 1 ? 0 : (pimple ? 5 : 1);
    if (S > 1 && nzl < gz) return fail(FY_ERR_INVALID, "slab thinner (%d planes) than the particle halo (%d)", nzl, gz);
    plane = (size_t)c->nx * c->ny;
    Nc = (int)(plane * nzl);
    nstore = plane * (size_t)(nzl + 2 * gz);
    Nglob = (int64_t)plane * c->nz;
    g.nx = c->nx; g.ny = c->ny; g.nz = nzl; g.Nc = Nc; g.gz = gz; g.c0 = (int)(plane * gz); g.kglob0 = comm->rank * nzl; g.nzglob = c->nz;
    g.dx = c->dx; g.Af = c->dx * c->dx; g.V = c->dx * c->dx * c->dx;
    g.graded = 0; g.h[0] = g.h[1] = g.h[2] = nullptr;
    total_volume = g.V * (double)Nglob;
    if (gradedc) {
        const double* hh[3] = {c->hx, c->hy, c->hz};
        const int nn[3] = {c->nx, c->ny, c->nz};
        double len[3] = {0, 0, 0};
        for (int a = 0; a < 3; ++a) {
            h_host[a].assign(hh[a], hh[a] + nn[a]);
            for (double v : h_host[a]) len[a] += v;
            FY_TRY(d_h[a].alloc_exact((size_t)nn[a]));
            FY_HIP(hipMemcpyAsync(d_h[a].p, hh[a], (size_t)nn[a] * sizeof(double), hipMemcpyHostToDevice, stream));
            g.h[a] = d_h[a].p;
        }
        FY_HIP(hipStreamSynchronize(stream));
        g.graded = 1;
        g.dx = std::cbrt((h_host[0][0] * h_host[1][0]) * h_host[2][0]);
        g.Af = g.dx * g.dx; g.V = g.dx * g.dx * g.dx;
        total_volume = (len[0] * len[1]) * len[2];
    }
    g.strip_B = g.strip_bp = g.strip_nzx = 0;
    {
        const int want = opt.strip_blocks;
        if (want != 0 && plane % 256 == 0 && nzl % 8 == 0) {
            const int bp = (int)(plane / 256);
            const int target = want > 0 ? want : std::max(1, (int)std::lround(8.0 * c->nx / 256.0));
            int best = 1;
            for (int d = 1; d <= bp; ++d) if (bp % d == 0 && std::abs(d - target) < std::abs(best - target)) best = d;
            g.strip_B = best; g.strip_bp = bp; g.strip_nzx = nzl / 8;
        }
    }
    g.upwind = c->convection_scheme;
    g.lim_twoByk = 2.0 / std::max(c->convection_limiter_k, 1e-15);
    g.rdx = 1.0 / g.dx; g.rhdx = 1.0 / (0.5 * g.dx); g.rV = 1.0 / g.V;
    g.pimple = pimple ? 1 : 0; g.dt = c->dt; g.nu = c->nu;
    bool need_ref = true;
    for (int q = 0; q < 6; ++q) {
        if (c->u_bc[q] != FY_BC_U_FIXED_VALUE && c->u_bc[q] != FY_BC_U_ZERO_GRADIENT && c->u_bc[q] != FY_BC_U_SLIP) return fail(FY_ERR_INVALID, "fy_solver_create: unknown velocity boundary type %d on side %d", c->u_bc[q], q);
        if (c->p_bc[q] != FY_BC_P_ZERO_GRADIENT && c->p_bc[q] != FY_BC_P_FIXED_VALUE && c->p_bc[q] != FY_BC_P_FIXED_FLUX) return fail(FY_ERR_INVALID, "fy_solver_create: unknown pressure boundary type %d on side %d", c->p_bc[q], q);
        g.u_bc[q] = c->u_bc[q]; g.p_bc[q] = c->p_bc[q]; g.p_val[q] = c->p_value[q];
        for (int a = 0; a < 3; ++a) g.u_val[q][a] = c->u_value[q][a];
        if (c->p_bc[q] == FY_BC_P_FIXED_VALUE) need_ref = false;
    }
    for (int a = 0; a < 3; ++a) g.g[a] = c->g[a];
    g.need_ref = need_ref ? 1 : 0; g.p_ref_cell = c->p_ref_cell; g.p_ref_value = c->p_ref_value;
    g.u_relax = c->u_relax;
    if (c->turbulence_model != FY_TURBULENCE_LAMINAR && c->turbulence_model != FY_TURBULENCE_SMAGORINSKY && c->turbulence_model != FY_TURBULENCE_KEQN && c->turbulence_model != FY_TURBULENCE_KEPSILON) return fail(FY_ERR_UNSUPPORTED, "fy_solver_create: unknown turbulence_model %d (DPMTurbulenceModels.C:67-77: laminar Stokes, RAS kEpsilon, LES Smagorinsky, LES kEqn)", c->turbulence_model);
    if (c->turbulence_model != FY_TURBULENCE_LAMINAR) {
        if (!pimple) return fail(FY_ERR_INVALID, "fy_solver_create: icoFoamYade has no turbulence model (icoFoamYade.C:79-85 is laplacian(nu, U))");
        if (!(c->les_ck > 0 && c->les_ce > 0 && c->les_delta_coeff > 0) || c->nut_initial < 0) return fail(FY_ERR_INVALID, "fy_solver_create: Smagorinsky needs Ck, Ce, deltaCoeff > 0 and nut >= 0");
        for (int q = 0; q < 6; ++q) {
            const bool has_k = c->turbulence_model == FY_TURBULENCE_KEQN || c->turbulence_model == FY_TURBULENCE_KEPSILON;
            if (c->nut_bc[q] != FY_BC_NUT_ZERO_GRADIENT && c->nut_bc[q] != FY_BC_NUT_FIXED_VALUE && !((c->nut_bc[q] == FY_BC_WALL_FUNCTION || c->nut_bc[q] == FY_BC_NUT_CALCULATED) && has_k))
                return fail(FY_ERR_INVALID, "fy_solver_create: unknown nut boundary type (nutkWallFunction / calculated need a model with a k equation)");
            g.nut_bc[q] = c->nut_bc[q]; g.nut_val[q] = c->nut_value[q];
        }
        les_delta = c->les_delta_coeff * std::pow(g.V, 1.0 / 3.0);
        {
            if (!(c->wf_kappa > 0 && c->wf_E > 0)) return fail(FY_ERR_INVALID, "fy_solver_create: wall-function constants kappa, E must be positive");
            g.wf_yPlusLam = wall_yplus_lam(c->wf_kappa, c->wf_E); g.wf_kappa = c->wf_kappa; g.wf_E = c->wf_E; g.wf_cmu25 = std::pow(c->ras_cmu, 0.25);
            g.nut_wall_live = 0;
            g.turb_model = c->turbulence_model; g.turb_ck = c->les_ck; g.turb_cmu = c->ras_cmu; g.turb_delta = les_delta; g.turb_dcoeff = c->les_delta_coeff;
            for (int q = 0; q < 6; ++q) {
                g.k_bc[q] = c->k_bc[q]; g.k_val[q] = c->k_value[q];
                g.eps_bc[q] = c->eps_bc[q] == FY_BC_NUT_FIXED_VALUE ? 1 : 0; g.eps_val[q] = c->eps_value[q];
            }
        }
        const bool keqn = c->turbulence_model == FY_TURBULENCE_KEQN, keps = c->turbulence_model == FY_TURBULENCE_KEPSILON;
        if (keqn || keps) {
            if (!(c->k_initial >= 0) || (keps && !(c->k_initial > 0)) || !(c->k_tol >= 0) || c->k_max_iter < 0 || c->k_relax > 1) return fail(FY_ERR_INVALID, "fy_solver_create: the k equation needs k >= 0 (> 0 for kEpsilon), a solver tolerance and a relaxation factor in (0, 1]");
// ... 238 lines not shown
    }
    FY_TRY(launch_reduce_finalize(stream, partials.p, Nc, nslots, courant ? ops_courant.p : nullptr, red_out.p));
    FY_TRY(comm->allreduce_ops(stream, red_out.p, nslots, courant ? 1u : 0u));
    double* land = (rb.mapped() && nslots <= 8) ? rb.host : h;
    FY_HIP(hipMemcpyAsync(land, red_out.p, nslots * sizeof(double), hipMemcpyDeviceToHost, stream));
    FY_HIP(hipStreamSynchronize(stream));
    if (land != h) for (int q = 0; q < nslots; ++q) h[q] = land[q];
    return FY_OK;
}
bool Solver::reduce_deferred(int nslots, bool courant, int* slot, int* rc, const int* ops) {
    *rc = FY_OK;
    if (!rb.mapped() || n_deferred + nslots > kDeferMax) return false;
    *slot = kDeferBase + n_deferred;
    n_deferred += nslots;
    if (comm->size == 1) {
        *rc = launch_reduce_finalize(stream, partials.p, Nc, nslots, ops ? ops : (courant ? ops_courant.p : nullptr), rb.dev + *slot);
        return true;
    }
    *rc = launch_reduce_finalize(stream, partials.p, Nc, nslots, ops ? ops : (courant ? ops_courant.p : nullptr), red_out.p);
    if (*rc == FY_OK) {
        *rc = comm->allreduce_ops(stream, red_out.p, nslots, ops ? 4u : (courant ? 1u : 0u));
    }
    if (*rc == FY_OK && hipMemcpyAsync(rb.slot(*slot), red_out.p, nslots * sizeof(double), hipMemcpyDeviceToHost, stream) != hipSuccess)
        *rc = fail(FY_ERR_HIP, "deferred read-back failed");
    return true;
}
int Solver::reduce_to_device(double* dst) {
    FY_TRY(launch_reduce_finalize(stream, partials.p, Nc, 1, nullptr, dst));
    return comm->allreduce(stream, dst, 1, false);
}

int Solver::solve_vec3(DevBuf<double>& X, const double* rhs, double tol, double rel_tol, int max_iter, int* iters, bool momentum, double* res0_out) {
    Comm::Tag tag(comm, momentum ? "momentum_solve" : "turbulence_solve");
    double h[6];
    if (momentum && usum_pending) {
        usum_pending = false;
        FY_HIP(hipStreamWaitEvent(stream, ev_usum1, 0));
    } else {
        FY_TRY(launch_sum3(stream, X.p + 3 * (size_t)g.c0, Nc, partials.p));
        FY_TRY(launch_reduce_finalize(stream, partials.p, Nc, 3, nullptr, xbar3.p));
        FY_TRY(comm->allreduce(stream, xbar3.p, 3, false));
    }
    double* xc = X.p; double* xn = xscr.p;
    double norm[3] = {1, 1, 1}, res0[3] = {0, 0, 0};
    int it = 0;
    for (;;) {
        const bool need_x = !(it == 0 && &X == &U && U_ghosts_fresh);
        kc[KC_MOM_PASS].begin(stream);
        const bool with_h = momentum && fused_corrector && cs.n_correctors > 0 && it >= 1;
        FY_TRY(overlapped(XW_MOMENTUM, need_x, [&](hipStream_t on) { return halo(xc, 3, plane, g.nz, g.gz, 1, on); }, [&](const FvGeo& gw) {
            return FVK(launch_mom_pass, stream, gw, M7(momentum), rhs, xc, xn, xbar3.p, (double)Nglob, partials.p, with_h ? src.p : nullptr, with_h ? rAU.p : nullptr,
                       with_h ? HbyA.p : nullptr);
        }));
        if (momentum) hbya_ready = with_h;
        kc[KC_MOM_PASS].end(stream);
        FY_TRY(reduce_read(6, false, h));
        if (vec3_converged(it, h, tol, rel_tol, norm, res0) || it >= max_iter) break;
        std::swap(xc, xn);
        ++it;
    }
    if (xc != X.p) {
        std::swap(X.p, xscr.p);
        if (&X == &U && cpl) cpl->c.dU = U.p;
    }
    if (&X == &U) U_ghosts_fresh = true;
    *iters = it;
    if (res0_out) *res0_out = res0[0];
    return FY_OK;
}

int Solver::corrector(bool final_inner) {
    Comm::Tag tag(comm, "corrector");
    if (hbya_ready) hbya_ready = false;
    else FY_TRY(overlapped(XW_CORRECTOR, !U_ghosts_fresh, [&](hipStream_t on) { return halo_U(on); },
                           [&](const FvGeo& gw) { return FVK(launch_HbyA, stream, gw, M7(), src.p, U.p, rAU.p, HbyA.p); }));
    if (!pimple && rAU_new) { FY_TRY(halo_cells(rAU, 1, 1)); if (face_arrays) FY_TRY(FVK(launch_interp_rAU, stream, g, rAU.p, F3(rAUf))); }
    MgLev& L = *mg[0];
    const bool fused_front = fused_corrector && !adjust_phi;
    const bool fused_back = fused_corrector;
    const bool ffc = faces_from_cells;
    if (fused_front) {
        clk_pres.begin(stream);
        FY_TRY(prepare_p_init(false));
        FY_TRY(overlapped(XW_CORRECTOR, true, [&](hipStream_t on) {
            comm->group_begin();
            FY_TRY(halo_cells(HbyA, 3, 1, on));
            FY_TRY(halo_p(on));
            return comm->group_end(on);
        }, [&](const FvGeo& gw) {
            return FVK(launch_corr_front, stream, gw, HbyA.p, U.p, C3(dcorr), C3(rAUf), C3(alphaf), C3(phiForces), F3(phiHbyA), F3(psn), rAU.p, alpha.p,  alpha.p,
                       L.A, prhs.p, rAU_new, p.p, p_sum_valid ? nullptr : sc.p + 6, p_sum, 1.0 / (double)Nglob, pr.p, partials.p, ffc);
        }));
    } else {
        FY_TRY(halo_cells(HbyA, 3, 1));
        FY_TRY(FVK(launch_phiHbyA, stream, g, HbyA.p, U.p, Uold.p, C3(phiOld), C3(rAUf), C3(alphaf), C3(phiForces), F3(phiHbyA), F3(psn), F3(ddtc), rAU_new ? 1 : 2));
        if (adjust_phi) {
            FY_TRY(FVK(launch_adjust_phi_sums, stream, g, C3(phiHbyA), C3(phiForces), partials.p));
            FY_TRY(launch_reduce_finalize(stream, partials.p, Nc, 4, nullptr, adj_sums.p));
            FY_TRY(comm->allreduce(stream, adj_sums.p, 4, false));
            FY_TRY(FVK(launch_adjust_phi_apply, stream, g, adj_sums.p, F3(phiHbyA), C3(phiForces), C3(rAUf), U.p, F3(psn), adj_err.p));
        }
        clk_pres.begin(stream);
    }
    for (int no = 0; no <= cs.n_non_orth_correctors; ++no) {
        const bool front_done = fused_front && no == 0;
        if (!front_done) FY_TRY(FVK(launch_assemble_pressure, stream, g, C3(phiHbyA), C3(rAUf), C3(alphaf), C3(psn), alpha.p,  alpha.p, L.A, prhs.p, rAU_new));
        if (rAU_new && L.distributed && comm->has_down() && !mg_deep) FY_TRY(FVK(launch_p_ghost_uz, stream, g, C3(rAUf), C3(alphaf), L.A));
        if (rAU_new) {
            if (comm->size == 1 && cs.p_solver == FY_PSOLVER_PCG_MG && mg.size() > 1) {
                FY_HIP(hipEventRecord(ev_assembled, stream));
                FY_HIP(hipStreamWaitEvent(comm_stream, ev_assembled, 0));
                std::swap(stream, comm_stream);
                coarse_on_side = true; coarse_marked = false;
                const int rc = build_coarse_operators();
                coarse_on_side = false;
                std::swap(stream, comm_stream);
                FY_TRY(rc);
                if (coarse_marked) { FY_HIP(hipEventRecord(ev_factor, comm_stream)); factor_pending = true; }
                else FY_HIP(hipEventRecord(ev_coarse, comm_stream));
                coarse_pending = true;
            } else {
                FY_TRY(build_coarse_operators());
            }
        }
        rAU_new = false;
        FY_TRY(solve_pressure(final_inner && no == cs.n_non_orth_correctors, front_done));
        FY_TRY(wait_factor());
        if (no == cs.n_non_orth_correctors && !fused_back) {
            FY_TRY(halo_p());
            FY_TRY(FVK(launch_flux_correct, stream, g, p.p, C3(phiHbyA), C3(rAUf), C3(alphaf), C3(psn), C3(phiForces), F3(pflux), F3(phi)));
            phi_fresh = true;
            if (pimple && p_relax_now > 0 && p_relax_now < 1) { FY_TRY(launch_relax_field(stream, p.p, pPrev.p, p_relax_now, nstore)); p_sum_valid = false; p_ghosts_fresh = false; }
        }
    }
    clk_pres.end(stream);
    double h[2];
    int slot = 0, rc = FY_OK;
    const bool diag_fused = fuse_diag && rb.mapped() && n_deferred + 4 <= kDeferMax;
    if (fused_back) {
        FY_TRY(overlapped(XW_CORRECTOR, !p_ghosts_fresh, [&](hipStream_t on) { return halo_p(on); }, [&](const FvGeo& gw) {
            return FVK(launch_corr_back, stream, gw, p.p, C3(phiHbyA), C3(rAUf), C3(alphaf), C3(psn), C3(phiForces), F3(phi), HbyA.p, rAU.p, U.p, alpha.p,
                        alpha.p, diag_fused ? partials.p : nullptr, ffc);
        }));
        phi_fresh = true;
        U_ghosts_fresh = false;
        if (pimple && p_relax_now > 0 && p_relax_now < 1) { FY_TRY(launch_relax_field(stream, p.p, pPrev.p, p_relax_now, nstore)); p_sum_valid = false; p_ghosts_fresh = false; }
        if (diag_fused) {
            if (!reduce_deferred(4, false, &slot, &rc, ops_diag.p)) return fail(FY_ERR_INVALID, "no room for the deferred diagnostics");
            FY_TRY(rc);
            cont_slots.push_back(slot);
            carry_slot = slot + 2;
            return FY_OK;
        }
        carry_slot = -1;
        if (pimple && !face_arrays) FY_TRY(FVK(launch_interp_alpha, stream, g, alpha.p, F3(alphaf)));
        FY_TRY(FVK(launch_cont_err, stream, g, C3(phi), C3(alphaf), alpha.p,  alpha.p, partials.p));
        if (reduce_deferred(2, false, &slot, &rc)) { FY_TRY(rc); cont_slots.push_back(slot); }
        else { FY_TRY(reduce_read(2, false, h)); note_cont_err(h); }
        return FY_OK;
    }
    if (diag_fused) {
        FY_TRY(FVK(launch_U_correct_diag, stream, g, HbyA.p, rAU.p, p.p, C3(psn), C3(phiForces), C3(pflux), C3(alphaf), C3(rAUf), U.p, C3(phi), alpha.p,
                                      alpha.p, partials.p));
        U_ghosts_fresh = false;
        if (!reduce_deferred(4, false, &slot, &rc, ops_diag.p)) return fail(FY_ERR_INVALID, "no room for the deferred diagnostics");
        FY_TRY(rc);
        cont_slots.push_back(slot);
        carry_slot = slot + 2;
        return FY_OK;
    }
    carry_slot = -1;
    FY_TRY(FVK(launch_cont_err, stream, g, C3(phi), C3(alphaf), alpha.p,  alpha.p, partials.p));
    if (reduce_deferred(2, false, &slot, &rc)) { FY_TRY(rc); cont_slots.push_back(slot); }
    else { FY_TRY(reduce_read(2, false, h)); note_cont_err(h); }
// ... 288 lines not shown
```

yade-openfoam-coupling_amd/csrc/fv_solver.hpp:

```cpp
#pragma once
#include <algorithm>
#include <cmath>
#include <memory>
#include <string>
#include <functional>
#include <vector>

#include "comm.hpp"
#include "coupling.hpp"
#include "field_average.hpp"
#include "fv_kernels.hpp"
#include "heat_exchange.hpp"

#define FVK(fn, ...) (g.graded ? ::fy::gr::fn(__VA_ARGS__) : ::fy::fn(__VA_ARGS__))

namespace fy {

constexpr int kMgCoarsest = kMgDirectMax, kMgCoarsestEdge = 8;
constexpr int kMgDeepGhost = 5;
constexpr int kMgReplicateBelow = 1 << 20;

struct MgLev {
    PMat A{};
    bool distributed = false;
    int gz = 0;
    size_t plane = 0;
    DevBuf<double> diag, ux, uy, uz, x0, x1, b;
    double* xcur = nullptr;
    double* xalt = nullptr;
    const double* bptr = nullptr;
};

struct Thermal {
    bool on = false;
    fy_thermal_desc d{};
    ScalarEqn eq{};
    DevBuf<double> T, Sp, Su;
    HeatExchange part;
    bool buoyant = false;
    DevBuf<double> buoy, usrc_sum;
    KernelClock clk_coeff, clk_flux, clk_asm, clk_buoy;
    int iters = 0;
    double res0 = 0.0;
    ~Thermal() { clk_coeff.destroy(); clk_flux.destroy(); clk_asm.destroy(); clk_buoy.destroy(); }
};

struct Solver {
    fy_case_desc cs{};
    std::vector<double> h_host[3];
    DevBuf<double> d_h[3];
    double total_volume = 0.0;
    FvGeo g{};
    int device = 0;
    hipStream_t stream = nullptr;
    hipStream_t comm_stream = nullptr;
    hipEvent_t ev_ready = nullptr, ev_halo = nullptr;
    hipEvent_t ev_fields = nullptr;
    hipEvent_t ev_assembled = nullptr, ev_coarse = nullptr, ev_factor = nullptr;
    hipEvent_t ev_usum0 = nullptr, ev_usum1 = nullptr;
    DevBuf<double> usum_partials;
    bool usum_pending = false;
    bool coarse_pending = false, factor_pending = false, coarse_on_side = false, coarse_marked = false;
    int wait_coarse() { if (coarse_pending) { coarse_pending = false; FY_HIP(hipStreamWaitEvent(stream, ev_coarse, 0)); } return FY_OK; }
    int wait_factor() { FY_TRY(wait_coarse()); if (factor_pending) { factor_pending = false; FY_HIP(hipStreamWaitEvent(stream, ev_factor, 0)); } return FY_OK; }
    fy_ctx* cpl = nullptr;
    bool pimple = false;
    int Nc = 0;
    size_t nstore = 0, plane = 0;
    int64_t Nglob = 0;
    Comm* comm = nullptr;
    SelfComm self_comm;

    DevBuf<double> U, Uold, p, alpha, uSource, uSourceDrag, uParticle, gradP, divT, vGrad, ddtU;
    DevBuf<double> nut;
    DevBuf<double> kturb, epsturb;
    TurbEqn eq_k{}, eq_eps{};
    double les_delta = 0.0;
    bool phi_fresh = true;
    CFace3 phi_now() const { return phi_fresh ? CFace3{{phi[0].p, phi[1].p, phi[2].p}} : CFace3{{phiOld[0].p, phiOld[1].p, phiOld[2].p}}; }
    bool rAU_new = true;
    DevBuf<double> phi[3], phiOld[3], psn[3], alphaf[3], phiHbyA[3], phiForces[3], rAUf[3], pflux[3], ddtc[3];
    DevBuf<double> dcorr[3];
    DevBuf<double> gradL;
    DevBuf<double> mbd;
    DevBuf<double> mdiag, man[6], src, rAU, HbyA, bmom, Gt, divG, xscr;
    std::vector<std::unique_ptr<MgLev> > mg;
    size_t mg_rep = 0;
    DevBuf<double> rep_stage;
    DevBuf<double> prhs, pr, pw, pp, ps, pzj;
    DevBuf<double> rep_gather;
    bool mg_deep = false;
    bool p_ghosts_fresh = false;
    bool U_ghosts_fresh = false;
    int halo_U(hipStream_t on = nullptr) { if (comm->size > 1 && !U_ghosts_fresh) { FY_TRY(halo_cells(U, 3, 1, on)); U_ghosts_fresh = true; } return FY_OK; }
    int halo_p(hipStream_t on = nullptr) { if (comm->size > 1 && !p_ghosts_fresh) { FY_TRY(halo_cells(p, 1, 1, on)); p_ghosts_fresh = true; } return FY_OK; }
    DevBuf<double> pPrev;
    double p_relax_now = 0.0;
    bool adjust_phi = false;
    DevBuf<double> adj_sums;
    DevBuf<int> adj_err;
    DevBuf<double> partials, red_out, sc, xbar3;
    bool hold_sources = false, sources_pending = false;
    bool overlap_halos = true;
    MappedReadback rb;
    DevBuf<int> ops_courant, ops_diag;
    fy_step_stats st{};
    double cumulative_cont_err = 0.0;
    EventTimer tim[4];
    KernelClock clk_mom, clk_pres;
    bool timing = true;
    enum { KC_MG_SMOOTH0 = 0, KC_P_APPLY_DOT, KC_MOM_PASS, KC_COUNT };
    KernelClock kc[KC_COUNT];

// ... 9 lines not shown
        clk_mom.destroy(); clk_pres.destroy();
        if (ev_ready) (void)hipEventDestroy(ev_ready);
        if (ev_halo) (void)hipEventDestroy(ev_halo);
        if (ev_fields) (void)hipEventDestroy(ev_fields);
        if (ev_assembled) (void)hipEventDestroy(ev_assembled);
        if (ev_usum0) (void)hipEventDestroy(ev_usum0);
        if (ev_usum1) (void)hipEventDestroy(ev_usum1);
        if (ev_coarse) (void)hipEventDestroy(ev_coarse);
        if (ev_factor) (void)hipEventDestroy(ev_factor);
        if (comm_stream) (void)hipStreamDestroy(comm_stream);
        if (stream) (void)hipStreamDestroy(stream);
    }

    int zero(DevBuf<double>& b) { if (b.n) FY_HIP(hipMemsetAsync(b.p, 0, b.n * sizeof(double), stream)); return FY_OK; }

    int halo(double* f, int ncomp, size_t pl, int nzl, int gzl, int w, hipStream_t on = nullptr) {
        if (comm->size == 1) return FY_OK;
        if (!on) on = stream;
        const size_t P = pl * (size_t)ncomp;
        double* own_lo = f + (size_t)gzl * P;
        double* own_hi = f + (size_t)(gzl + nzl - w) * P;
        double* gh_lo = f + (size_t)(gzl - w) * P;
        double* gh_hi = f + (size_t)(gzl + nzl) * P;
        return comm->neighbour_exchange(on, own_hi, gh_lo, own_lo, gh_hi, (size_t)w * P);
    }
    int halo_cells(DevBuf<double>& f, int ncomp, int w, hipStream_t on = nullptr) { return halo(f.p, ncomp, plane, g.nz, g.gz, w, on); }

    bool can_window() const { return comm->size > 1 && overlap_halos && plane % 256 == 0 && g.nz >= 3; }
    FvGeo window(int ka, int kb) const {
        FvGeo w = g;
        const int bp = (int)(plane / 256);
        w.red_stride = red_blocks(Nc);
        w.win_blk0 = ka * bp;
        w.win_nblk = (kb >= g.nz ? w.red_stride : kb * bp) - w.win_blk0;
        return w;
    }
    enum { XW_STEP = 0, XW_PARTICLE, XW_MOMENTUM, XW_CORRECTOR, XW_COUNT };
    KernelClock clk_xwait[XW_COUNT];
    bool xwait_timing = false;
    double xwait_ms[XW_COUNT] = {0, 0, 0, 0};
    template <class X, class L>
    int overlapped(int phase, bool needed, X&& xchg, L&& launch) {
        if (!needed || comm->size == 1) return launch(g);
        KernelClock& ck = clk_xwait[phase];
        if (!can_window()) {
            ck.begin(stream);
            FY_TRY(xchg(stream));
            ck.end(stream);
            return launch(g);
        }
        FY_HIP(hipEventRecord(ev_ready, stream));
        FY_TRY(launch(window(1, g.nz - 1)));
        FY_HIP(hipStreamWaitEvent(comm_stream, ev_ready, 0));
        FY_TRY(xchg(comm_stream));
        FY_HIP(hipEventRecord(ev_halo, comm_stream));
        ck.begin(stream);
        FY_HIP(hipStreamWaitEvent(stream, ev_halo, 0));
        ck.end(stream);
        FY_TRY(launch(window(0, 1)));
        return launch(window(g.nz - 1, g.nz));
    }
    int halo_level(MgLev& L, double* x) { return L.distributed ? halo(x, 1, L.plane, L.A.nz, L.gz, 1) : FY_OK; }

    int create(const fy_case_desc* c, const fy_transport* tr, int dev, Comm* cm);

    int reduce_read(int nslots, bool courant, double* h);
    static constexpr int kDeferBase = 8, kDeferMax = 2 + 4 * 255;
    int n_deferred = 0;
    bool reduce_deferred(int nslots, bool courant, int* slot, int* rc, const int* ops = nullptr);
    int reduce_to_device(double* dst);

    int solve_momentum(int* iters) { return solve_vec3(U, bmom.p, cs.u_tol, cs.u_rel_tol, cs.u_max_iter, iters, true); }
    int solve_vec3(DevBuf<double>& X, const double* rhs, double tol, double rel_tol, int max_iter, int* iters, bool momentum = false, double* res0_out = nullptr);

    int smooth(size_t l, MgLev& L, double w, bool with_dot = false);
    PMat slice_of(const MgLev& L, const MgLev& Cc) const;
    static constexpr double kMgWa = 1.7318685872766142, kMgWb = 0.5695012757370842;
    MgWeights mgw{2, {kMgWa, kMgWb, 0, 0}};
    int vcycle(size_t l);
    PMat planes_of(const MgLev& L, int ext, int* kofs = nullptr) const;
    int vcycle_deep(size_t l, int E);
    int exchange_operator_ghosts(MgLev& L);
    bool want_vcycle_dot = false, vcycle_dot_done = false;
    static constexpr int kMgCoarseSweeps = 120;
    int coarse_sweeps = kMgCoarseSweeps;
    bool fuse_prolong = true;
    int ref_cell_at(size_t lvl, const PMat& A, int k0) const;
    int build_coarse_operators();
    DevBuf<double> mg_inv, mg_ref;
    double p_sum = 0.0;
    bool p_sum_valid = false;
    int solve_pressure(bool final_iter, bool init_done = false);
    int precondition(const double* r_host, double* z_host);
    int prepare_p_init(bool with_halo = true);
    bool fused_corrector = true;
    bool hbya_ready = false;
    bool face_arrays = true;
    bool faces_from_cells = true;

    int corrector(bool final_inner);
    bool fuse_diag = true;
    int carry_slot = -1;
    bool carry_valid = false;
    double carry_h[2] = {0, 0};

    std::vector<int> cont_slots;
    int courant_slot = -1;
    void note_cont_err(const double* h) {
        const double tv = total_volume;
        st.cont_err_sum_local = cs.dt * h[0] / tv; st.cont_err_global = cs.dt * h[1] / tv;
        cumulative_cont_err += st.cont_err_global; st.cont_err_cumulative = cumulative_cont_err;
    }
    void note_courant(const double* h) { st.courant_max = 0.5 * h[0] * cs.dt; st.courant_mean = 0.5 * (h[1] / total_volume) * cs.dt; }
    int turbulence_correct();
    int st_k_iters = 0;

    int step();
    FieldAverage avg;
    const double* avg_source(const std::string& name, int* comp) const;
    int set_field_average(const fy_average_desc* d);
    Monitors mon;
    DevBuf<double> Vcell, bndP, bndU, bndT, d_Tval;
    DevBuf<int> d_Tbc;
    int t_patch(TPatch* out);
    int set_monitors(const fy_monitor_desc* d);
    Thermal th;
    int thermal_create(const fy_case_desc* c);
    int heat_coefficients();
    int solve_temperature();
    int heat_fluxes();
    int buoyancy();
    const double* momentum_source() const { return th.buoyant ? th.usrc_sum.p : uSource.p; }
    int set_particle_temperatures(int batch, const double* tp, bool on_device);
    int get_particle_thermal_state(int batch, double* tp, int64_t* resets);
    int get_particle_heat(int batch, double* q);
    int thermal_stats(int32_t* iterations, double* initial_residual, double* heat_to_particles_W);
    int field(const char* name, double** ptr, size_t* count);
};

}

struct fy_solver { fy::Solver s; };
```

Before: 206.4.

## Fuse first Jacobi smoothing sweep into residual-producing kernels for MG V-cycle

Kernels that produce a residual (pressure init, fused corrector front, PCG update, MG residual-restrict) now also write the first damped-Jacobi iterate w0*r/diag into the level's alternate buffer. The V-cycle then runs a single smooth from that iterate instead of the two-sweeps-from-zero kernel. This saves one pass over the matrix and vectors per non-distributed level, at the cost of an extra store and a diag load in the producer kernels. It is gated by an env flag and by the previous solve's iteration count, so the extra write is skipped on the last PCG iteration.

```diff
diff --git a/yade-openfoam-coupling_amd/csrc/common.hpp b/yade-openfoam-coupling_amd/csrc/common.hpp
--- a/yade-openfoam-coupling_amd/csrc/common.hpp
+++ b/yade-openfoam-coupling_amd/csrc/common.hpp
@@ -34,6 +34,7 @@
     bool faces_from_arrays;
     bool no_pairs;
     bool no_tail_cache;
+    bool no_first_iterate;
     int ipc_slot_kb;
 };
 Options options();
diff --git a/yade-openfoam-coupling_amd/csrc/coupling.cpp b/yade-openfoam-coupling_amd/csrc/coupling.cpp
--- a/yade-openfoam-coupling_amd/csrc/coupling.cpp
+++ b/yade-openfoam-coupling_amd/csrc/coupling.cpp
@@ -48,6 +48,7 @@
     q.faces_from_arrays = on("FOAMYADE_FACES_FROM_ARRAYS");
     q.no_pairs = on("FOAMYADE_NO_PAIRS");
     q.no_tail_cache = on("FOAMYADE_NO_TAIL_CACHE");
+    q.no_first_iterate = on("FOAMYADE_NO_FIRST_ITERATE");
     q.ipc_slot_kb = (int)num("FOAMYADE_IPC_SLOT_KB", 0);
     g_kernel_flags.store((q.no_pairs ? 1 : 0) | (q.no_tail_cache ? 2 : 0) | (q.locate_wide ? 4 : 0), std::memory_order_relaxed);
     return q;
diff --git a/yade-openfoam-coupling_amd/csrc/fv_kernels.hip b/yade-openfoam-coupling_amd/csrc/fv_kernels.hip
--- a/yade-openfoam-coupling_amd/csrc/fv_kernels.hip
+++ b/yade-openfoam-coupling_amd/csrc/fv_kernels.hip
@@ -1376,7 +1376,7 @@
                                                     FaceSrc rAUf, FaceSrc alphaf, CFace3 phiForces, Face3 phiHbyA, Face3 psn,
                                                     const double* __restrict__ rAU, const double* __restrict__ alpha, const double* __restrict__ alphaOld, PMat A,
                                                     double* __restrict__ rhs, const double* __restrict__ x, const double* __restrict__ xbar_dev, double xsum_val,
-                                                    double inv_n, double* __restrict__ res, double* __restrict__ partials) {
+                                                    double inv_n, double* __restrict__ res, double* __restrict__ partials, double* __restrict__ x1, double w0) {
     double v[2] = {0, 0};
     const double xbar = (xbar_dev ? xbar_dev[0] : xsum_val) * inv_n;
     FY_RED_LOOP_G(g, t) {
@@ -1463,6 +1463,7 @@
         const double Aref = rs * xbar;
         const double rr = r - Ax;
         res[c] = rr;
+        if (x1) x1[c] = w0 * rr / (STORE_A ? dg : A.diag[c]);
         v[0] += fabs(rr);
         v[1] += fabs(Ax - Aref) + fabs(r - Aref);
     }
@@ -1740,11 +1741,12 @@
 
 int launch_corr_front(hipStream_t s, FvGeo g, const double* HbyA, const double* U, CFace3 dcorr, CFace3 rAUf, CFace3 alphaf, CFace3 phiForces, Face3 phiHbyA,
                       Face3 psn, const double* rAU, const double* alpha, const double* alphaOld, PMat A, double* rhs, bool store_A, const double* x,
-                      const double* xsum_dev, double xsum_val, double inv_n, double* res, double* partials, bool faces_from_cells) {
+                      const double* xsum_dev, double xsum_val, double inv_n, double* res, double* partials, bool faces_from_cells, double* x1, double w0) {
     const FaceSrc rs{rAUf, faces_from_cells ? rAU : nullptr}, as{alphaf, faces_from_cells ? alpha : nullptr};
     const dim3 grid(fv_red_grid(g)), blk(256);
+    if (x1 && (x1 == res || x1 == rhs || x1 == x)) return fail(FY_ERR_INVALID, "fused corrector sweep: the first iterate needs a buffer of its own");
 #define FY_FRONT(SA, FC) hipLaunchKernelGGL((k_corr_front<SA, FC>), grid, blk, 0, s, g, HbyA, U, dcorr, rs, as, phiForces, phiHbyA, psn, rAU, alpha, alphaOld, A, rhs, \
-                                            x, xsum_dev, xsum_val, inv_n, res, partials)
+                                            x, xsum_dev, xsum_val, inv_n, res, partials, x1, w0)
     if (store_A) { if (faces_from_cells) FY_FRONT(true, true); else FY_FRONT(true, false); }
     else { if (faces_from_cells) FY_FRONT(false, true); else FY_FRONT(false, false); }
 #undef FY_FRONT
diff --git a/yade-openfoam-coupling_amd/csrc/fv_kernels_api.inc b/yade-openfoam-coupling_amd/csrc/fv_kernels_api.inc
--- a/yade-openfoam-coupling_amd/csrc/fv_kernels_api.inc
+++ b/yade-openfoam-coupling_amd/csrc/fv_kernels_api.inc
@@ -47,7 +47,7 @@
                      const double* HbyA, const double* rAU, double* U, const double* alpha, const double* alphaOld, double* partials, bool faces_from_cells);
 int launch_corr_front(hipStream_t s, FvGeo g, const double* HbyA, const double* U, CFace3 dcorr, CFace3 rAUf, CFace3 alphaf, CFace3 phiForces, Face3 phiHbyA,
                       Face3 psn, const double* rAU, const double* alpha, const double* alphaOld, PMat A, double* rhs, bool store_A, const double* x,
-                      const double* xsum_dev, double xsum_val, double inv_n, double* res, double* partials, bool faces_from_cells);
+                      const double* xsum_dev, double xsum_val, double inv_n, double* res, double* partials, bool faces_from_cells, double* x1 = nullptr, double w0 = 0.0);
 
 
 int launch_p_ghost_uz(hipStream_t s, FvGeo g, CFace3 rAUf, CFace3 alphaf, PMat A);
diff --git a/yade-openfoam-coupling_amd/csrc/fv_linalg_kernels.hip b/yade-openfoam-coupling_amd/csrc/fv_linalg_kernels.hip
--- a/yade-openfoam-coupling_amd/csrc/fv_linalg_kernels.hip
+++ b/yade-openfoam-coupling_amd/csrc/fv_linalg_kernels.hip
@@ -97,7 +97,7 @@
 }
 
 __global__ __launch_bounds__(256) void k_p_init(PMat A, const double* __restrict__ b, const double* __restrict__ x, const double* __restrict__ xbar_dev,
-                                                double xsum_val, double inv_n, double* __restrict__ r, double* __restrict__ partials) {
+                                                double xsum_val, double inv_n, double* __restrict__ r, double* __restrict__ partials, double* __restrict__ x1, double w0) {
     double v[2] = {0, 0};
     const double xbar = (xbar_dev ? xbar_dev[0] : xsum_val) * inv_n;
     FY_RED_LOOP(t, A.N) {
@@ -106,6 +106,7 @@
         const double Aref = p_rowsum(A, c) * xbar;
         const double rr = b[c] - Ax;
         r[c] = rr;
+        if (x1) x1[c] = w0 * rr / A.diag[c];
         v[0] += fabs(rr);
         v[1] += fabs(Ax - Aref) + fabs(b[c] - Aref);
     }
@@ -123,7 +124,7 @@
 template <bool FIRST>
 __global__ __launch_bounds__(256) void k_pcg_cg_update(int n, int c0, const double* __restrict__ u, const double* __restrict__ w, double* __restrict__ p,
                                                        double* __restrict__ sv, double* __restrict__ x, double* __restrict__ r, double* __restrict__ sc, int it,
-                                                       double* __restrict__ partials) {
+                                                       double* __restrict__ partials, const double* __restrict__ diag, double* __restrict__ x1, double w0) {
     double v[2] = {0, 0};
     const double gamma = sc[0], delta = sc[1];
     double beta = 0.0, al = gamma / delta;
@@ -144,6 +145,7 @@
         x[c] = xn;
         const double rr = r[c] - al * sn;
         r[c] = rr;
+        if (x1) x1[c] = w0 * rr / diag[c];
         v[0] += fabs(rr);
         v[1] += xn;
     }
@@ -275,7 +277,7 @@
 }
 
 __global__ __launch_bounds__(256) void k_mg_residual_restrict(PMat A, const double* __restrict__ b, const double* __restrict__ x, PMat C,
-                                                              double* __restrict__ bc) {
+                                                              double* __restrict__ bc, double* __restrict__ x1c, double w0) {
     const int tc = blockIdx.x * 256 + threadIdx.x;
     if (tc >= C.N) return;
     const int I = tc % C.nx, q = tc / C.nx, J = q % C.ny, K = q / C.ny;
@@ -292,10 +294,11 @@
         }
     }
     bc[tc + C.c0] = acc;
+    if (x1c) x1c[tc + C.c0] = w0 * acc / C.diag[tc + C.c0];
 }
 
 __global__ __launch_bounds__(256) void k_mg_residual_restrict_tiled(PMat A, const double* __restrict__ b, const double* __restrict__ x, PMat C,
-                                                                    double* __restrict__ bc) {
+                                                                    double* __restrict__ bc, double* __restrict__ x1c, double w0) {
     __shared__ double r[2][2][64];
     const int tx = threadIdx.x & 63, ty = (threadIdx.x >> 6) & 1, tz = threadIdx.x >> 7;
     const int i = blockIdx.x * 64 + tx, j = blockIdx.y * 2 + ty, k = blockIdx.z * 2 + tz;
@@ -310,8 +313,10 @@
         const int I = blockIdx.x * 32 + (int)threadIdx.x, J = blockIdx.y, K = blockIdx.z;
         if (I < C.nx) {
             const int q = 2 * (int)threadIdx.x;
-            bc[C.c0 + I + C.nx * (J + C.ny * K)] = ((r[0][0][q] + r[0][0][q + 1]) + (r[0][1][q] + r[0][1][q + 1])) +
-                                                   ((r[1][0][q] + r[1][0][q + 1]) + (r[1][1][q] + r[1][1][q + 1]));
+            const int cc = C.c0 + I + C.nx * (J + C.ny * K);
+            const double acc = ((r[0][0][q] + r[0][0][q + 1]) + (r[0][1][q] + r[0][1][q + 1])) + ((r[1][0][q] + r[1][0][q + 1]) + (r[1][1][q] + r[1][1][q + 1]));
+            bc[cc] = acc;
+            if (x1c) x1c[cc] = w0 * acc / C.diag[cc];
         }
     }
 }
@@ -409,7 +414,7 @@
 template <bool FIRST>
 __global__ __launch_bounds__(128) void k_pcg_cg_update2(int n, int c0, const double* __restrict__ u, const double* __restrict__ w, double* __restrict__ p,
                                                         double* __restrict__ sv, double* __restrict__ x, double* __restrict__ r, double* __restrict__ sc, int it,
-                                                        double* __restrict__ partials) {
+                                                        double* __restrict__ partials, const double* __restrict__ diag, double* __restrict__ x1, double w0) {
     double2 v[2] = {make_double2(0, 0), make_double2(0, 0)};
     const double gamma = sc[0], delta = sc[1];
     double beta = 0.0, al = gamma / delta;
@@ -432,6 +437,7 @@
         st2(x + c, xa, xb);
         const double ra = ro.x - al * sn.x, rb = ro.y - al * sn.y;
         st2(r + c, ra, rb);
+        if (x1) { const double2 dg = ld2(diag + c); st2(x1 + c, w0 * ra / dg.x, w0 * rb / dg.y); }
         v[0] = make_double2(fabs(ra), fabs(rb));
         v[1] = make_double2(xa, xb);
     }
@@ -502,7 +508,7 @@
 }
 template <int PX, int TY, int TZ>
 __global__ __launch_bounds__(256) void k_mg_residual_restrict_tiled2(PMat A, const double* __restrict__ b, const double* __restrict__ x, PMat C,
-                                                                     double* __restrict__ bc) {
+                                                                     double* __restrict__ bc, double* __restrict__ x1c, double w0) {
     static_assert(PX * TY * TZ == 256 && TY % 2 == 0 && TZ % 2 == 0, "tile shape");
     __shared__ double r[TZ][TY][PX];
     const int tx = threadIdx.x % PX, ty = (threadIdx.x / PX) % TY, tz = threadIdx.x / (PX * TY);
@@ -520,8 +526,12 @@
     if ((int)threadIdx.x < NC) {
         const int cx = threadIdx.x % PX, cy = (threadIdx.x / PX) % (TY / 2), cz = threadIdx.x / (PX * (TY / 2));
         const int I = blockIdx.x * PX + cx, J = blockIdx.y * (TY / 2) + cy, K = blockIdx.z * (TZ / 2) + cz;
-        if (I < C.nx && J < C.ny && K < C.nz)
-            bc[C.c0 + I + C.nx * (J + C.ny * K)] = (r[2 * cz][2 * cy][cx] + r[2 * cz][2 * cy + 1][cx]) + (r[2 * cz + 1][2 * cy][cx] + r[2 * cz + 1][2 * cy + 1][cx]);
+        if (I < C.nx && J < C.ny && K < C.nz) {
+            const int cc = C.c0 + I + C.nx * (J + C.ny * K);
+            const double acc = (r[2 * cz][2 * cy][cx] + r[2 * cz][2 * cy + 1][cx]) + (r[2 * cz + 1][2 * cy][cx] + r[2 * cz + 1][2 * cy + 1][cx]);
+            bc[cc] = acc;
+            if (x1c) x1c[cc] = w0 * acc / C.diag[cc];
+        }
     }
 }
 
@@ -903,8 +913,9 @@
     return FY_OK;
 }
 
-int launch_p_init(hipStream_t s, PMat A, const double* b, const double* x, const double* xsum_dev, double xsum_val, double inv_n, double* r, double* partials) {
-    hipLaunchKernelGGL(k_p_init, dim3(red_blocks(A.N)), dim3(256), 0, s, A, b, x, xsum_dev, xsum_val, inv_n, r, partials);
+int launch_p_init(hipStream_t s, PMat A, const double* b, const double* x, const double* xsum_dev, double xsum_val, double inv_n, double* r, double* partials,
+                  double* x1, double w0) {
+    hipLaunchKernelGGL(k_p_init, dim3(red_blocks(A.N)), dim3(256), 0, s, A, b, x, xsum_dev, xsum_val, inv_n, r, partials, x1, w0);
     FY_LAUNCH_CHECK();
     return FY_OK;
 }
@@ -915,13 +926,15 @@
     return FY_OK;
 }
 
-int launch_pcg_cg_update(hipStream_t s, int n, int c0, const double* u, const double* w, double* p, double* sv, double* x, double* r, double* sc, int it, double* partials) {
-    if (pairs_ok(n, c0) && al16(u) && al16(w) && al16(p) && al16(sv) && al16(x) && al16(r)) {
-        if (it == 0) hipLaunchKernelGGL(k_pcg_cg_update2<true>, dim3(red_blocks(n)), dim3(128), 0, s, n, c0, u, w, p, sv, x, r, sc, it, partials);
-        else hipLaunchKernelGGL(k_pcg_cg_update2<false>, dim3(red_blocks(n)), dim3(128), 0, s, n, c0, u, w, p, sv, x, r, sc, it, partials);
-    }
-    else if (it == 0) hipLaunchKernelGGL(k_pcg_cg_update<true>, dim3(red_blocks(n)), dim3(256), 0, s, n, c0, u, w, p, sv, x, r, sc, it, partials);
-    else hipLaunchKernelGGL(k_pcg_cg_update<false>, dim3(red_blocks(n)), dim3(256), 0, s, n, c0, u, w, p, sv, x, r, sc, it, partials);
+int launch_pcg_cg_update(hipStream_t s, int n, int c0, const double* u, const double* w, double* p, double* sv, double* x, double* r, double* sc, int it, double* partials,
+                         const double* diag, double* x1, double w0) {
+    if (x1 && (!diag || x1 == u || x1 == w || x1 == p || x1 == sv || x1 == x || x1 == r)) return fail(FY_ERR_INVALID, "PCG update: the first iterate needs a buffer of its own");
+    if (pairs_ok(n, c0) && al16(u) && al16(w) && al16(p) && al16(sv) && al16(x) && al16(r) && al16(diag) && al16(x1)) {
+        if (it == 0) hipLaunchKernelGGL(k_pcg_cg_update2<true>, dim3(red_blocks(n)), dim3(128), 0, s, n, c0, u, w, p, sv, x, r, sc, it, partials, diag, x1, w0);
+        else hipLaunchKernelGGL(k_pcg_cg_update2<false>, dim3(red_blocks(n)), dim3(128), 0, s, n, c0, u, w, p, sv, x, r, sc, it, partials, diag, x1, w0);
+    }
+    else if (it == 0) hipLaunchKernelGGL(k_pcg_cg_update<true>, dim3(red_blocks(n)), dim3(256), 0, s, n, c0, u, w, p, sv, x, r, sc, it, partials, diag, x1, w0);
+    else hipLaunchKernelGGL(k_pcg_cg_update<false>, dim3(red_blocks(n)), dim3(256), 0, s, n, c0, u, w, p, sv, x, r, sc, it, partials, diag, x1, w0);
     FY_LAUNCH_CHECK();
     return FY_OK;
 }
@@ -1031,22 +1044,23 @@
     return FY_OK;
 }
 
-int launch_mg_residual_restrict(hipStream_t s, PMat A, const double* b, const double* x, PMat C, double* bc) {
+int launch_mg_residual_restrict(hipStream_t s, PMat A, const double* b, const double* x, PMat C, double* bc, double* x1c, double w0) {
+    if (x1c && (x1c == bc || x1c == x || x1c == b)) return fail(FY_ERR_INVALID, "restriction: the coarse first iterate needs a buffer of its own");
     if (C.N > 8192 && C.ny * 2 >= A.ny && C.nz * 2 >= A.nz) {
         if (pairs_ok(A) && al16(b) && al16(x) && A.ny % 2 == 0 && A.nz % 2 == 0) {
             const int px_opts[4] = {64, 32, 16, 8};
             int best = 64; double best_fill = 0.0;
             for (int px : px_opts) { const double fill = (double)A.nx / (double)(div_up(A.nx, 2 * px) * 2 * px); if (fill > best_fill + 1e-9) { best_fill = fill; best = px; } }
-            if (best == 64) hipLaunchKernelGGL((k_mg_residual_restrict_tiled2<64, 2, 2>), dim3(div_up(A.nx, 128), div_up(A.ny, 2), div_up(A.nz, 2)), dim3(256), 0, s, A, b, x, C, bc);
-            else if (best == 32) hipLaunchKernelGGL((k_mg_residual_restrict_tiled2<32, 4, 2>), dim3(div_up(A.nx, 64), div_up(A.ny, 4), div_up(A.nz, 2)), dim3(256), 0, s, A, b, x, C, bc);
-            else if (best == 16) hipLaunchKernelGGL((k_mg_residual_restrict_tiled2<16, 4, 4>), dim3(div_up(A.nx, 32), div_up(A.ny, 4), div_up(A.nz, 4)), dim3(256), 0, s, A, b, x, C, bc);
-            else hipLaunchKernelGGL((k_mg_residual_restrict_tiled2<8, 8, 4>), dim3(div_up(A.nx, 16), div_up(A.ny, 8), div_up(A.nz, 4)), dim3(256), 0, s, A, b, x, C, bc);
-        }
-        else hipLaunchKernelGGL(k_mg_residual_restrict_tiled, dim3(div_up(A.nx, 64), C.ny, C.nz), dim3(256), 0, s, A, b, x, C, bc);
+            if (best == 64) hipLaunchKernelGGL((k_mg_residual_restrict_tiled2<64, 2, 2>), dim3(div_up(A.nx, 128), div_up(A.ny, 2), div_up(A.nz, 2)), dim3(256), 0, s, A, b, x, C, bc, x1c, w0);
+            else if (best == 32) hipLaunchKernelGGL((k_mg_residual_restrict_tiled2<32, 4, 2>), dim3(div_up(A.nx, 64), div_up(A.ny, 4), div_up(A.nz, 2)), dim3(256), 0, s, A, b, x, C, bc, x1c, w0);
+            else if (best == 16) hipLaunchKernelGGL((k_mg_residual_restrict_tiled2<16, 4, 4>), dim3(div_up(A.nx, 32), div_up(A.ny, 4), div_up(A.nz, 4)), dim3(256), 0, s, A, b, x, C, bc, x1c, w0);
+            else hipLaunchKernelGGL((k_mg_residual_restrict_tiled2<8, 8, 4>), dim3(div_up(A.nx, 16), div_up(A.ny, 8), div_up(A.nz, 4)), dim3(256), 0, s, A, b, x, C, bc, x1c, w0);
+        }
+        else hipLaunchKernelGGL(k_mg_residual_restrict_tiled, dim3(div_up(A.nx, 64), C.ny, C.nz), dim3(256), 0, s, A, b, x, C, bc, x1c, w0);
         FY_LAUNCH_CHECK();
         return FY_OK;
     }
-    hipLaunchKernelGGL(k_mg_residual_restrict, dim3(div_up(C.N, 256)), dim3(256), 0, s, A, b, x, C, bc);
+    hipLaunchKernelGGL(k_mg_residual_restrict, dim3(div_up(C.N, 256)), dim3(256), 0, s, A, b, x, C, bc, x1c, w0);
     FY_LAUNCH_CHECK();
     return FY_OK;
 }
diff --git a/yade-openfoam-coupling_amd/csrc/fv_linalg_kernels.hpp b/yade-openfoam-coupling_amd/csrc/fv_linalg_kernels.hpp
--- a/yade-openfoam-coupling_amd/csrc/fv_linalg_kernels.hpp
+++ b/yade-openfoam-coupling_amd/csrc/fv_linalg_kernels.hpp
@@ -25,9 +25,10 @@
 int launch_p_apply(hipStream_t s, PMat A, const double* x, double* y);
 int launch_p_apply_dot(hipStream_t s, PMat A, const double* x, const double* r , double* y, double* partials);
 int launch_p_init(hipStream_t s, PMat A, const double* b, const double* x, const double* xsum_dev , double xsum_val, double inv_n,
-                  double* r, double* partials);
+                  double* r, double* partials, double* x1 = nullptr, double w0 = 0.0);
 int launch_dot(hipStream_t s, int n, int c0, const double* a, const double* b , double* partials);
-int launch_pcg_cg_update(hipStream_t s, int n, int c0, const double* u, const double* w, double* p, double* sv, double* x, double* r, double* sc, int it, double* partials);
+int launch_pcg_cg_update(hipStream_t s, int n, int c0, const double* u, const double* w, double* p, double* sv, double* x, double* r, double* sc, int it, double* partials,
+                         const double* diag = nullptr, double* x1 = nullptr, double w0 = 0.0);
 int launch_jacobi_precond(hipStream_t s, PMat A, const double* r, double* z);
 int launch_mg_coarsen(hipStream_t s, PMat F, PMat C, int ref_c = -1, const double* ref_term = nullptr);
 int launch_mg_ref_term(hipStream_t s, PMat A0, int ref_local, double* out);
@@ -35,7 +36,7 @@
 int launch_mg_smooth_two_from_zero(hipStream_t s, PMat A, const double* b, double* xn, double w, double w2);
 int launch_mg_smooth(hipStream_t s, PMat A, const double* b, const double* x, double* xn, double w);
 int launch_mg_smooth_dot(hipStream_t s, PMat A, const double* b, const double* x, double* xn, double w, double* partials);
-int launch_mg_residual_restrict(hipStream_t s, PMat A, const double* b, const double* x, PMat C, double* bc);
+int launch_mg_residual_restrict(hipStream_t s, PMat A, const double* b, const double* x, PMat C, double* bc, double* x1c = nullptr, double w0 = 0.0);
 int launch_mg_prolong_add(hipStream_t s, PMat A, double* x, PMat C, const double* xc);
 int launch_mg_prolong_add_planes(hipStream_t s, PMat A , int kofs , double* x, PMat C, const double* xc);
 int launch_mg_smooth_prolong(hipStream_t s, PMat A, const double* b, const double* x, PMat C, const double* xc, double* xn, double w);
diff --git a/yade-openfoam-coupling_amd/csrc/fv_pressure.cpp b/yade-openfoam-coupling_amd/csrc/fv_pressure.cpp
--- a/yade-openfoam-coupling_amd/csrc/fv_pressure.cpp
+++ b/yade-openfoam-coupling_amd/csrc/fv_pressure.cpp
@@ -100,12 +100,25 @@
     return FY_OK;
 }
 
+bool Solver::tail_from(size_t l) const {
+    const MgLev& L = *mg[l];
+    return !L.distributed && L.A.N <= kMgTailCells && mg.size() - l <= (size_t)kMgTailMax;
+}
+
+double* Solver::first_iterate_slot(size_t l) {
+    MgLev& L = *mg[l];
+    L.first_in_alt = first_iterate && cs.p_solver == FY_PSOLVER_PCG_MG && !L.distributed && l + 1 < mg.size() && !tail_from(l);
+    return L.first_in_alt ? L.xalt : nullptr;
+}
+
 int Solver::vcycle(size_t l) {
     const double w = 0.8;
     const MgWeights& W = mgw;
     if (l >= 1) FY_TRY(wait_coarse());
     MgLev& L = *mg[l];
-    if (!L.distributed && L.A.N <= kMgTailCells && mg.size() - l <= (size_t)kMgTailMax) {
+    const bool have_first = L.first_in_alt;
+    L.first_in_alt = false;
+    if (tail_from(l)) {
         FY_TRY(wait_factor());
         PMat A[kMgTailMax]; double* x0[kMgTailMax]; double* x1[kMgTailMax]; double* b[kMgTailMax];
         const int n = (int)(mg.size() - l);
@@ -125,7 +138,8 @@
     }
     MgLev& Cc = *mg[l + 1];
     if (!L.distributed) {
-        FY_TRY(launch_mg_smooth_two_from_zero(stream, L.A, L.bptr, L.xcur, W.w[0], W.w[1]));
+        if (have_first) FY_TRY(launch_mg_smooth(stream, L.A, L.bptr, L.xalt, L.xcur, W.w[1]));
+        else FY_TRY(launch_mg_smooth_two_from_zero(stream, L.A, L.bptr, L.xcur, W.w[0], W.w[1]));
     } else {
         FY_TRY(launch_mg_smooth_first(stream, L.A, L.bptr, L.xcur, W.w[0]));
         FY_TRY(smooth(l, L, W.w[1]));
@@ -138,7 +152,8 @@
         FY_TRY(launch_mg_residual_restrict(stream, L.A, L.bptr, L.xcur, loc, rep_stage.p));
         FY_TRY(comm->allgather(stream, rep_stage.p, Cc.b.p, (size_t)loc.N));
     } else {
-        FY_TRY(launch_mg_residual_restrict(stream, L.A, L.bptr, L.xcur, Cc.A, Cc.b.p));
+        double* const x1c = L.distributed ? nullptr : first_iterate_slot(l + 1);
+        FY_TRY(launch_mg_residual_restrict(stream, L.A, L.bptr, L.xcur, Cc.A, Cc.b.p, x1c, W.w[0]));
     }
     Cc.bptr = Cc.b.p;
     FY_TRY(vcycle(l + 1));
@@ -233,7 +248,8 @@
     double h[2];
     if (!init_done) {
         FY_TRY(prepare_p_init());
-        FY_TRY(launch_p_init(stream, L.A, prhs.p, p.p, p_sum_valid ? nullptr : sc.p + 6, p_sum, 1.0 / (double)Nglob, pr.p, partials.p));
+        double* const x1 = p_iters_last[final_iter] >= 1 ? first_iterate_slot(0) : nullptr;
+        FY_TRY(launch_p_init(stream, L.A, prhs.p, p.p, p_sum_valid ? nullptr : sc.p + 6, p_sum, 1.0 / (double)Nglob, pr.p, partials.p, x1, mgw.w[0]));
     }
     FY_TRY(reduce_read(2, false, h));
     const double norm = h[1] + 1e-20;
@@ -263,7 +279,8 @@
             kc[KC_P_APPLY_DOT].end(stream);
             FY_TRY(launch_reduce_finalize(stream, partials.p, Nc, 2, nullptr, sc.p));
             FY_TRY(comm->allreduce(stream, sc.p, 2, false));
-            FY_TRY(launch_pcg_cg_update(stream, Nc, g.c0, u, pw.p, pp.p, ps.p, p.p, pr.p, sc.p, it, partials.p));
+            double* const x1 = (cs.p_solver == FY_PSOLVER_PCG_MG && !mg_deep && it + 1 < p_iters_last[final_iter]) ? first_iterate_slot(0) : nullptr;
+            FY_TRY(launch_pcg_cg_update(stream, Nc, g.c0, u, pw.p, pp.p, ps.p, p.p, pr.p, sc.p, it, partials.p, L.A.diag, x1, mgw.w[0]));
             if (it == 0) {
                 std::swap(ps.p, pw.p);
                 if (u == L.xcur) {
@@ -280,6 +297,8 @@
             p_sum = h[1]; p_sum_valid = true;
         } while (++it < cs.p_max_iter && !converged(res));
     }
+    L.first_in_alt = false;
+    p_iters_last[final_iter] = it;
     st.p_final_residual = res;
     st.p_iters_total += it; st.p_solves += 1;
     return FY_OK;
@@ -297,6 +316,7 @@
         const bool want = want_vcycle_dot, done = vcycle_dot_done;
         FY_HIP(hipMemcpyAsync(pzj.p + g.c0, r_host, bytes, hipMemcpyHostToDevice, stream));
         L.bptr = pzj.p;
+        L.first_in_alt = false;
         int rc;
         if (mg_deep) rc = vcycle_deep(0, 1);
         else { want_vcycle_dot = true; rc = vcycle(0); }
diff --git a/yade-openfoam-coupling_amd/csrc/fv_solver.cpp b/yade-openfoam-coupling_amd/csrc/fv_solver.cpp
--- a/yade-openfoam-coupling_amd/csrc/fv_solver.cpp
+++ b/yade-openfoam-coupling_amd/csrc/fv_solver.cpp
@@ -36,6 +36,7 @@
     const Options opt = options();
     overlap_halos = opt.halo_overlap;
     fused_corrector = !opt.no_fused_corrector;
+    first_iterate = !opt.no_first_iterate;
     faces_from_cells = !opt.faces_from_arrays;
     comm->set_aux_stream(comm_stream);
     const int S = comm->size;
@@ -440,6 +441,8 @@
     if (fused_front) {
         clk_pres.begin(stream);
         FY_TRY(prepare_p_init(false));
+        const bool final_first = final_inner && cs.n_non_orth_correctors == 0;
+        double* const x1 = p_iters_last[final_first] >= 1 ? first_iterate_slot(0) : nullptr;
         FY_TRY(overlapped(XW_CORRECTOR, true, [&](hipStream_t on) {
             comm->group_begin();
             FY_TRY(halo_cells(HbyA, 3, 1, on));
@@ -447,7 +450,7 @@
             return comm->group_end(on);
         }, [&](const FvGeo& gw) {
             return FVK(launch_corr_front, stream, gw, HbyA.p, U.p, C3(dcorr), C3(rAUf), C3(alphaf), C3(phiForces), F3(phiHbyA), F3(psn), rAU.p, alpha.p,  alpha.p,
-                       L.A, prhs.p, rAU_new, p.p, p_sum_valid ? nullptr : sc.p + 6, p_sum, 1.0 / (double)Nglob, pr.p, partials.p, ffc);
+                       L.A, prhs.p, rAU_new, p.p, p_sum_valid ? nullptr : sc.p + 6, p_sum, 1.0 / (double)Nglob, pr.p, partials.p, ffc, x1, mgw.w[0]);
         }));
     } else {
         FY_TRY(halo_cells(HbyA, 3, 1));
diff --git a/yade-openfoam-coupling_amd/csrc/fv_solver.hpp b/yade-openfoam-coupling_amd/csrc/fv_solver.hpp
--- a/yade-openfoam-coupling_amd/csrc/fv_solver.hpp
+++ b/yade-openfoam-coupling_amd/csrc/fv_solver.hpp
@@ -29,6 +29,7 @@
     double* xcur = nullptr;
     double* xalt = nullptr;
     const double* bptr = nullptr;
+    bool first_in_alt = false;
 };
 
 struct Thermal {
@@ -204,6 +205,10 @@
     int vcycle_deep(size_t l, int E);
     int exchange_operator_ghosts(MgLev& L);
     bool want_vcycle_dot = false, vcycle_dot_done = false;
+    bool first_iterate = true;
+    bool tail_from(size_t l) const;
+    double* first_iterate_slot(size_t l);
+    int p_iters_last[2] = {1 << 20, 1 << 20};
     static constexpr int kMgCoarseSweeps = 120;
     int coarse_sweeps = kMgCoarseSweeps;
     bool fuse_prolong = true;
```

After: 208.0, median of 6. No clear change (+0.8%).
